# YuQiao0303/PointDreamer

Hardware: AMD Instinct MI355X
Metric: shapes/hour (30k-pt cloud, 8x256^2 views, DDNM) on MI355X (higher is better)
Workload: dtype f16 (f32 accumulate; f32 GroupNorm/softmax statistics, f32 geometry); 1 GPU; configs[2]: synthetic 30k-point sphere shape, 8x256^2 views, texture_gen_method='DDNM_inpaint' (100 DDNM steps, 552.8M-param guided-diffusion UNet, random-init weights), NBF [21], atlas 1024^2, complete_unseen_by='unproject', optimize_from=None, hidden-point removal on (device); 4 independent shapes per step, their views batched through the UNet together; parallelism=shapes-parallel x1, views_per_unet_batch=32

## Files before the change

include/pdhip.h:

```cpp
#ifndef PDHIP_H
#define PDHIP_H
#include <stdint.h>
#include <stddef.h>
#ifdef __cplusplus
extern "C" {
#endif

#define PDHIP_OK 0
#define PDHIP_E_ARG (-1)
#define PDHIP_E_HIP (-2)
#define PDHIP_E_STATE (-3)
#define PDHIP_E_NOMEM (-4)
#define PDHIP_E_UNKNOWN_NAME (-5)

int pdhip_version(void);
int pdhip_lab_build(void);
const char* pdhip_last_error(void);
int pdhip_debug_carve_log(int on);
int pdhip_debug_carve_log_read(uint64_t* triples, int capacity);

int pdhip_project_points(const float* cam_params, int V, const float* vertices, int Vn,
                         const float* points, int N, int rescale, double padding,
                         float* pos , float* vertice_uvs ,
                         float* uv_centers, float* uv_scales,
                         float* point_uvs , float* point_depths ,
                         uint32_t* minmax_ws, void* stream);

int pdhip_raster_mesh(const float* pos , int V, int Vn, const int32_t* faces , int F,
                      int R, uint64_t* zkey_ws, uint8_t* hard_masks, int64_t* face_idxs, float* depths,
                      void* stream);
size_t pdhip_raster_mesh_ws_bytes(int V, int F, int R);
int pdhip_raster_mesh_ws(const float* pos, int V, int Vn, const int32_t* faces, int F, int R, uint64_t* zkey_ws, size_t ws_bytes,
                         uint8_t* hard_masks, int64_t* face_idxs, float* depths, void* stream);
int pdhip_debug_set_raster_path(int path);

int pdhip_raster_barycentrics(const float* pos , int V, int Vn, const int32_t* faces, int R,
                              const int64_t* face_idxs , float* bary , void* stream);
int pdhip_interpolate(const float* attr , int C, const int32_t* tri , const int64_t* face_idxs,
                      const float* bary, long long pixels, float* out , void* stream);

int pdhip_shade_views(const int64_t* face_idxs , const float* bary , int V, int R, const float* attr ,
                      int Na, int C, const int32_t* tri , int F, const float* atlas , int A,
                      const float* face_normals , const float* cam_params ,
                      const float* light_dirs , int L, int double_side, double gamma, float* images ,
                      uint8_t* rgba , void* stream);

int pdhip_shade_views_materials(const int64_t* face_idxs , const float* bary , int V, int R,
                                const float* uvs , int T, const int64_t* face_uvs_idx ,
                                const int32_t* face_material , int F,
                                const uint8_t* texels , int64_t texel_bytes, const int64_t* mat_offset ,
                                const int32_t* mat_wh , const float* mat_kd , int M,
                                const float* face_normals , const float* cam_params ,
                                const float* light_dirs , int L, int double_side, double gamma,
                                float* images , uint8_t* rgba ,
                                int32_t* material_idx , void* stream);

size_t pdhip_image_metrics_workspace_bytes(int N, int H, int W);
int pdhip_image_metrics(const uint8_t* a, const uint8_t* b, int N, int H, int W, int C, int gaussian, uint64_t* sse ,
                        double* ssim , void* ws, void* stream);

size_t pdhip_uv_atlas_ws_bytes(int Vn, int F);
int pdhip_uv_atlas(const float* vertices , int Vn, const int64_t* faces , int F, int resolution, int gutter,
                   float* uvs , int64_t* tex_idx , int32_t* face_chart ,
                   int32_t* counts ,
                   void* ws, void* stream);

size_t pdhip_estimate_normals_ws_bytes(int N, int k, int n_eyes);
int pdhip_estimate_normals(const float* points , int N, int k, int n_eyes, double eye_radius, float* normals ,
                           int32_t* counts , void* ws, void* stream);
size_t pdhip_surface_recon_ws_bytes(int N, int depth);
int pdhip_surface_recon(const float* points , const float* normals , const float* colors , int N, int depth,
                        float* vertices, int vertex_capacity, int64_t* faces, int face_capacity, float* vertex_colors ,
                        int32_t* counts , float* info , void* ws, void* stream);

size_t pdhip_simplify_mesh_workspace_bytes(int Vn, int F);
int pdhip_simplify_mesh(const float* vertices , int Vn, const int64_t* faces , int F, const float* vertex_colors ,
                        int target_faces, float* out_vertices , int64_t* out_faces , float* out_colors ,
                        int32_t* counts , void* ws, void* stream);

size_t pdhip_sample_mesh_workspace_bytes(int F, int N);
int pdhip_sample_mesh(const float* vertices , int Vn, const int64_t* faces , int F, const float* uvs , int T,
                      const int64_t* face_uvs_idx , const int32_t* face_material ,
                      const uint8_t* face_keep , const uint8_t* texels , int64_t texel_bytes,
                      const int64_t* mat_offset , const int32_t* mat_wh , const float* mat_kd , int M,
                      const float* rand , int N, float* coords , float* colors , float* normals ,
                      float* uvs_out , int32_t* face_idx , int32_t* material_idx , void* ws, void* stream);

int pdhip_project_points_shapes(const float* cam_params , int V, int S, const float* vertices , int Vn,
                                const float* points , int N, int rescale, double padding, float* pos ,
                                float* vertice_uvs, float* uv_centers , float* uv_scales , float* point_uvs ,
                                float* point_depths , uint32_t* minmax_ws , void* stream);
int pdhip_raster_mesh_shapes(const float* pos , int V, int S, int Vn, const int32_t* faces , int F, int R,
                             uint64_t* zkey_ws, size_t ws_bytes , uint8_t* hard_masks,
                             int64_t* face_idxs, float* depths, void* stream);
int pdhip_hidden_point_removal_shapes(const float* points , int N, const double* eyes , int V, int S, double radius,
                                      const uint8_t* skip , uint8_t* visibility ,
                                      void* ws , void* stream);
int pdhip_sparse_views_shapes(const int64_t* point_pixels , const float* colors , const uint8_t* validation,
                              const uint8_t* hard_masks, int V, int S, int N, int res, int point_size, int edge_point_size,
                              double mask_ratio_thresh, float* sparse, float* mask0, float* mask2, float* scale_factors ,
                              float* mask_ratios, void* ws , void* stream);
int pdhip_texel_visibility_shapes(const float* cam_params, int V, int S, const float* gb_pos , const uint8_t* mask ,
                                  int A, const float* uv_centers, const float* uv_scales, double padding, const float* mesh_depths ,
                                  int R, float offset, uint8_t* visibility , void* stream);
int pdhip_nbf_shrink_shapes(const uint8_t* mask , const uint8_t* visibility , int V, int S, int A,
                            const int32_t* kernels, int K, uint8_t* out , uint8_t* ws , void* stream);
int pdhip_view_select_blend_shapes(const float* cam_params, int V, int S, const float* gb_pos, const uint8_t* mask, const int64_t* face_id,
                                   int A, const float* f_normals , int F, const float* base_dirs , const float* uv_centers,
                                   const float* uv_scales, double padding, const float* scale_factors, const uint8_t* shrinked ,
                                   int K, const uint8_t* visibility, int complete_unseen_by_projection, const float* inpainted ,
                                   int r, float* atlas , uint8_t* painted , int32_t* view_ids ,
                                   void* stream);

int pdhip_rescale_vertices(float* pos , int V, int Vn, const float* uv_centers, const float* uv_scales,
                           const float* factors , double padding, void* stream);
size_t pdhip_optimize_color_ws_bytes(int V, int res, int A);
int pdhip_optimize_color(float* atlas, int A, const float* uv_map, const int64_t* face_idxs, int V, int res,
                         const float* inpainted , int r, const uint8_t* shrinked, double lr, int iterations,
                         float* final_images, void* ws, void* stream);

int pdhip_resize_mask(const uint8_t* in , int B, int in_h, int in_w,
                      uint8_t* out , int out_h, int out_w, void* stream);

int pdhip_point_visibility(int cam_res, const float* point_uvs , const float* point_depths ,
                           const float* mesh_depths , int V, int N, float offset,
                           uint8_t* visibility , int64_t* point_pixels , void* stream);

size_t pdhip_hpr_ws_bytes(int V, int N);
int pdhip_hidden_point_removal(const float* points , int N, const double* eyes , int V, double radius,
                               const uint8_t* skip, uint8_t* visibility, void* ws, void* stream);
int pdhip_hpr_read_counters(const void* ws, int V, long long* out , void* stream);

int pdhip_point_pixels(const float* point_uvs , int V, int N, int res,
                       int64_t* point_pixels , void* stream);
int pdhip_point_visibility_pixels(int cam_res, const float* point_uvs, const float* point_depths, const float* mesh_depths,
                                  int V, int N, float offset, uint8_t* visibility , int res,
                                  int64_t* point_pixels , void* stream);

size_t pdhip_sparse_views_ws_bytes(int V, int N, int res);
int pdhip_sparse_views(const int64_t* point_pixels , const float* colors ,
                       const uint8_t* validation , const uint8_t* hard_masks ,
                       int V, int N, int res, int point_size, int edge_point_size, double mask_ratio_thresh,
                       float* sparse , float* mask0, float* mask2,
                       float* scale_factors , float* mask_ratios ,
                       void* ws, void* stream);

size_t pdhip_nearest_fill_ws_ints(int B, int H, int W);
int pdhip_nearest_fill(const float* img, float* out, int B, int C, int H, int W,
                       int64_t batch_stride, int64_t chan_stride, int64_t pix_stride,
                       const void* mask, int mask_is_f32, int64_t mask_batch_stride,
                       int32_t* ws, void* stream);

size_t pdhip_linear_fill_ws_bytes(int B, int H, int W);
int pdhip_linear_fill(const float* img, float* out, int B, int C, int H, int W, const void* mask, int mask_is_f32,
                      int64_t mask_batch_stride, void* ws, int32_t* tri, void* stream);
int pdhip_linear_fill_unresolved(const void* ws, int B, int H, int W, int* out, void* stream);
int pdhip_debug_set_linear_local(int on);

int pdhip_debug_set_unproject_generic(int on);

int pdhip_texel_visibility(const float* cam_params, int V, const float* gb_pos ,
                           const uint8_t* mask , int A, const float* uv_centers ,
                           const float* uv_scales , double padding,
                           const float* mesh_depths , int R, float offset,
                           uint8_t* visibility, void* stream);

int pdhip_nbf_shrink(const uint8_t* mask , const uint8_t* visibility , int V, int A,
                     const int32_t* kernels, int K, uint8_t* out, uint8_t* ws, void* stream);
int pdhip_pack_bits(const uint8_t* in , long long n, uint64_t* out , void* stream);
int pdhip_unpack_bits(const uint64_t* in , long long n, uint8_t* out , void* stream);
int pdhip_nbf_triptych(const uint8_t* mask, const uint8_t* visibility, int V, int A, int kernel, uint8_t* out, uint8_t* ws,
                       void* stream);

int pdhip_view_select_blend(const float* cam_params, int V, const float* gb_pos, const uint8_t* mask,
                            const int64_t* face_id , int A, const float* f_normals ,
                            const float* base_dirs , const float* uv_centers, const float* uv_scales,
                            double padding, const float* scale_factors ,
                            const uint8_t* shrinked, int K, const uint8_t* visibility,
                            int complete_unseen_by_projection,
                            const float* inpainted , int r,
                            float* atlas, uint8_t* painted, int32_t* view_ids, void* stream);

int pdhip_compact_texels(const float* gb_pos, const uint8_t* mask, int A, const int32_t* view_ids,
                         float* points, int64_t* coords, int64_t* point_view_ids, int32_t* count_dev,
                         int32_t* ws, void* stream);

typedef struct pdhip_unet pdhip_unet;

int pdhip_unet_create(int image_size, int model_channels, int num_res_blocks, const int* channel_mult, int n_mult,
                      const int* attention_ds, int n_att, int num_head_channels, int out_channels, int max_batch,
                      pdhip_unet** out);
void pdhip_unet_destroy(pdhip_unet* u);
long long pdhip_unet_arena_bytes(const pdhip_unet* u);
int pdhip_unet_route_table(int image_size, int model_channels, int num_res_blocks, const int* channel_mult, int n_mult, const int* attention_ds,
                           int n_att, int num_head_channels, int out_channels, int max_batch, int N, char* buf, int buf_len);
int pdhip_unet_num_tensors(const pdhip_unet* u);
int pdhip_unet_load_tensor(pdhip_unet* u, const char* name, const void* data, int is_f16, const int64_t* shape, int ndim,
                           void* stream);
int pdhip_unet_missing_tensors(const pdhip_unet* u, char* buf, int buf_len);
int pdhip_unet_forward(pdhip_unet* u, const float* x, const float* t, int N, float* out, void* stream);
int pdhip_unet_profile(pdhip_unet* u, int enable);
int pdhip_unet_profile_read(pdhip_unet* u, double* total_ms, double* total_flops, long long* launches);
int pdhip_unet_profile_read_attention(pdhip_unet* u, double* total_ms, double* total_flops, long long* launches);

int pdhip_ddnm_schedule(float* at, float* at_next, int* t, int* t_next, float* coefs);
int pdhip_ddnm_prepare(const float* masked_imgs , const float* masks , float* y, int N, int HW, void* stream);
int pdhip_ddnm_step(float* x, const float* et, int et_channels, const float* y, const float* mask, const float* eps,
                    uint64_t seed, int step, int N, int HW, void* stream);
int pdhip_ddnm_sample(pdhip_unet* u, const float* masked_imgs, const float* masks, int N, const float* x_T,
                      const float* eps_tape, uint64_t seed, int n_steps, float* out, void* stream);
int pdhip_ddnm_sample_keyed(pdhip_unet* u, const float* masked_imgs, const float* masks, int N, const float* x_T,
                            const float* eps_tape, uint64_t seed, uint64_t first_image_key, int n_steps, float* out, void* stream);

int pdhip_debug_set_conv_bk(int bk);
int pdhip_debug_set_conv_tile(int geometry);
int pdhip_debug_set_conv_stages(int stages);
int pdhip_debug_set_conv_splitk(void* ws, long long ws_floats, int splits);
int pdhip_debug_set_conv_halo_strips(int mode);
int pdhip_pack_conv_weight_f16(const float* w_oihw, int Cout, int Cin, int taps, void* w_packed , void* stream);
int pdhip_conv2d_nhwc_f16(const void* x, const void* w_packed , const float* bias, const void* residual,
                          void* y, int N, int H, int W, int Cin, int Cout, int Cout_pad, int taps, const void* zero_page,
                          void* stream);
int pdhip_groupnorm_nhwc_f16(const void* x, const float* gamma, const float* beta, const float* film , int N,
                             int H, int W, int C, int silu, int resample, void* y, float* stats_ws, float* ws,
                             long long ws_floats, void* stream);
int pdhip_gn_silu_conv3x3_nhwc_f16(const void* x, const float* gamma, const float* beta, const float* film ,
                                   long long film_stride, const void* w_packed, const float* bias, const void* residual, void* y,
                                   int N, int H, int W, int Cin, int Cout, int Cout_pad, const void* zero_page, float* ws,
                                   long long ws_floats, void* stream);
int pdhip_debug_conv3x3_apply(const void* x, const float* table , const void* w_packed, const float* bias, const void* residual,
                              void* y, int N, int H, int W, int Cin, int Cout, int Cout_pad, const void* zero_page, void* stream);
int pdhip_debug_set_fold_skip(int on);
int pdhip_debug_set_up_phase(int mode);
int pdhip_pack_conv_up2_phase_f16(const void* w_packed, int Cin, int Cout_pad, void* w_phase, void* stream);
int pdhip_conv3x3_up2_phase_nhwc_f16(const void* x, const void* w_phase, const float* bias, void* y, int N, int H, int W, int Cin, int Cout,
                                     int Cout_pad, const void* zero_page, float* gn_part, void* stream);
int pdhip_conv3x3_up2_halo_nhwc_f16(const void* x, const void* w_packed, const float* bias, void* y, int N, int H, int W, int Cin, int Cout,
                                    int Cout_pad, const void* zero_page, void* stream);
int pdhip_debug_set_fold_resample(int on);
int pdhip_debug_set_fold_finalize(int max_batch);
int pdhip_debug_set_fold_finalize_chunks(int chunks);
int pdhip_debug_set_conv_sk(int mode, int tile, int splits);
int pdhip_debug_set_conv_sk_stages(int stages);
int pdhip_debug_set_conv_sk_kgroups(int kg);
int pdhip_debug_set_attn(int nbuf, int vt_form, int qtiles);
int pdhip_debug_set_conv_sk_order(int order);
int pdhip_gn_silu_skip1x1_nhwc_f16(const void* xa, const void* xb, int Ca, int C, const float* stats, const float* gamma, const float* beta,
                                   const void* w_packed, const float* bias, void* h0, void* sk, int N, int H, int W, void* stream);
int pdhip_debug_set_gn_iters(int iters);
int pdhip_debug_set_gn_skip_variant(int v);
int pdhip_debug_set_fuse_skip(int mode, int min_tiles);
int pdhip_debug_set_fuse_gn(int on);
int pdhip_mark_unpainted_faces(const int64_t* face_id, const uint8_t* painted, int A, int F, uint8_t* flags , void* stream);
int pdhip_vertex_texel_fetch(const float* vert_uvs , int V, const float* atlas , const uint8_t* mask ,
                             int A, int32_t* texel , float* colors , float* count , void* stream);
int pdhip_neighbor_diffuse_round(const int32_t* rowptr , const int32_t* colidx, int V, const int32_t* invalid, int IV,
                                 float* colors, float* count, float* tmp , int* colored, void* stream);
int pdhip_scatter_vertex_colors(const int32_t* texel, const float* colors, int V, float* atlas, uint8_t* mask,
                                int32_t* owner_ws , int A, void* stream);
size_t pdhip_subdivide_with_uv_ws_bytes(int V, int U, int F, int K);
int pdhip_subdivide_with_uv(const float* vertices , int V, const int64_t* faces , int F, const float* uvs , int U,
                            const int64_t* face_uv_idx , const int64_t* face_index , int K,
                            float* out_vertices, int64_t* out_faces, float* out_uvs, int64_t* out_face_uv_idx,
                            int32_t* counts , int32_t* counts_host , void* ws, void* stream);
size_t pdhip_vertex_uv_table_ws_bytes(int V, int F);
int pdhip_vertex_uv_table(int V, const int64_t* faces , const int64_t* face_uv_idx , int F, const float* uvs ,
                          int U, float* vert_uvs , int32_t* counts , void* ws, void* stream);
size_t pdhip_neighbour_csr_ws_bytes(int V, int F);
int pdhip_neighbour_csr(int V, const int64_t* faces , int F, int32_t* rowptr , int32_t* colidx ,
                        int32_t* counts , int32_t* counts_host , void* ws, void* stream);
size_t pdhip_compact_zero_count_ws_bytes(int V);
int pdhip_compact_zero_count(const float* count , int V, int32_t* invalid , int32_t* counts ,
                             int32_t* counts_host , void* ws, void* stream);

long long pdhip_io_ply_count(const char* path);
int pdhip_io_read_ply_xyzrgb(const char* path, float* xyz , uint8_t* rgb , long long n);
int pdhip_io_write_obj_mtl(const char* obj_path, const char* mtl_path, const char* texture_stem, const double* points, long long P,
                           const double* tcoords, long long T, const int64_t* faces, const int64_t* facetex, long long F);
int pdhip_io_write_obj_plain(const char* obj_path, const float* points , long long P, const int64_t* faces , long long F);
int pdhip_io_write_png(const char* path, const uint8_t* hwc, int H, int W, int channels, int zlib_level);
int pdhip_chw_f32_to_hwc_u8(const float* img, int C, int H, int W, uint8_t* out, void* stream);

size_t pdhip_unet_head_ws_floats(int N, int H, int W, int C, int Cout);
int pdhip_unet_head_f32(const void* x, const float* gamma, const float* beta, const float* w_oihw, const float* bias,
                        int N, int H, int W, int C, int Cout, float* y_nchw, float* ws, long long ws_floats, void* stream);
int pdhip_conv_rr_f16(const void* x, const void* x2, int C, int Ca, int gn_mode, const float* gamma, const float* beta, const float* film,
                      long long film_stride, const float* partA, int chunksA, const float* partB, int chunksB, const void* xs, const void* xs2, int Cs,
                      int Cs1, int taps, const void* wf, const float* bias, const void* residual, int res_up, void* y, int N, int H, int W, int Cout,
                      float* ws, long long ws_floats, float* gn_part, int* gn_chunks, void* stream);
long long pdhip_conv_rr_weight_halfs(int Cin, int taps, int Cs, int Cout);
int pdhip_conv_rr_pack_f16(const void* w_packed, int Cin, int taps, int Cs, int Cout, void* wf, void* stream);
int pdhip_gn_octet_partials_f16(const void* x, int N, int HW, int C, int chunks, float* part, void* stream);
int pdhip_gn_apply_parts_f16(const void* x, const void* x2, int Ca, int C, const float* partA, int chunksA, const float* partB, int chunksB, const float* gamma,
                             const float* beta, const float* film, long long film_stride, int N, int H, int W, int silu, void* y, void* stream);
int pdhip_debug_conv_launch_nhwc_f16(const void* x, const void* x2, int Cin1, const void* w_packed, const float* bias, const void* residual, int res_up,
                                     const void* xs, const void* xs2, int Cs1, int Cs, void* y, int N, int H, int W, int Cin, int Cout, int Cout_pad, int taps,
                                     const void* zero_page, float* ws, long long ws_floats, float* gn_part, long long gn_part_floats, int* gn_chunks, int* kernel,
                                     void* stream);
int pdhip_gn_finalize_oct_f32(const float* partA, int Ca, int chunksA, const float* partB, int Cb, int chunksB, int N, int HW, float* stats, void* stream);
int pdhip_conv_ht_f16(const void* x, const void* w_packed, const float* bias, const void* residual, int res_up, void* y, int N, int H, int W, int Cin, int Cout,
                      int Cout_pad, const void* zero_page, float* splitk_ws, long long splitk_ws_floats, float* gn_part, int* gn_chunks, void* stream);
int pdhip_conv_ht_plan(int N, int H, int W, int Cin, int Cout, int Cout_pad, long long splitk_ws_floats, int* routed, int* slabs);
int pdhip_debug_set_conv_ht(int mode, int slabs);
int pdhip_debug_set_rr_gn(int max_width);
int pdhip_debug_set_conv_rr(int mode, int variant, int slabs);
int pdhip_attention_f16(const void* qkv , void* out , int N, int T, int C, int head_dim,
                        void* vt_ws , void* stream);
int pdhip_philox_normal(float* out, long long n, uint64_t seed, uint64_t stream_id, void* stream);
int pdhip_gemv_rows_f32(const float* W, const float* b, const float* x, float* y, int R, int K, int N, int silu_out, void* stream);
int pdhip_timestep_mlp_f32(const float* t, int N, int mc, const float* w0, const float* b0, const float* w2, const float* b2, float* emb_silu,
                           float* tmp, void* stream);
int pdhip_conv_in_f16(const float* x_nchw, const void* Wt, const float* bias, void* Y, int N, int H, int W, int Cout, int Cout_pad, void* im2col_ws,
                      const void* zero_page, void* stream);
int pdhip_gn_apply_f16(const void* x, const void* x2, int Ca, int C, const float* stats, const float* partA, int chunksA, const float* partB, int chunksB,
                       const float* gamma, const float* beta, const float* film, long long film_stride, int N, int H, int W, int silu, int resample, void* y,
                       void* y_raw, void* stream);
int pdhip_gn_table_f32(const float* stats, const float* gamma, const float* beta, const float* film, long long film_stride, int N, int C, float* table, void* stream);
int pdhip_resample2x_nhwc_f16(const void* x, int N, int H, int W, int C, int mode, void* y, void* stream);
int pdhip_concat_channels_f16(const void* a, int Ca, const void* b, int Cb, long long pixels, void* y, void* stream);
int pdhip_bench_copy16(const void* src, void* dst, long long bytes, int blocks, int unroll, void* stream);

size_t pdhip_nearest_points_workspace_bytes(int Q, int M);
int pdhip_nearest_points_stage_chunk(void);
int pdhip_nearest_points(const float* queries, int Q, const float* targets, int M, double* d2, int32_t* idx, int32_t* counts, void* ws, void* stream);
int pdhip_debug_set_nearest_path(int path);
size_t pdhip_cloud_metrics_workspace_bytes(int T);
int pdhip_cloud_metrics(const double* d2, const int32_t* idx, int Q, const float* normals_src, const float* normals_tgt, int M,
                        const double* thresholds, int T, double* sums, int64_t* within, void* ws, void* stream);

size_t pdhip_mesh_contains_workspace_bytes(int Vn, int F, int Q, int resolution);
int pdhip_mesh_contains(const float* vertices, int Vn, const int64_t* faces, int F, const float* points, int Q, int resolution, uint8_t* occ,
                        int32_t* counts, void* ws, void* stream);
int pdhip_debug_set_mesh_contains_slabs(int slabs);
int pdhip_occupancy_iou(const uint8_t* a, const uint8_t* b, int Q, int64_t* out, void* stream);

size_t pdhip_closest_on_mesh_workspace_bytes(int Vn, int F, int Q);
int pdhip_closest_on_mesh(const float* vertices, int Vn, const int64_t* faces, int F, const float* points, int Q, double* d2, int32_t* face,
                          double* closest, int32_t* counts, void* ws, void* stream);
int pdhip_debug_set_closest_on_mesh(int cells_per_axis, int path);

size_t pdhip_fps_workspace_bytes(int N, int M);
int pdhip_fps(const float* points, int N, int M, int start, int32_t* idx, double* min_d2, int32_t* counts, void* ws, void* stream);
int pdhip_debug_set_fps_cells(int cells_per_axis);
size_t pdhip_owner_mean_colors_workspace_bytes(int M);
int pdhip_owner_mean_colors(const int32_t* owner, const float* colors, int N, int M, const float* fallback, float* out, void* ws_or_null, void* stream);

size_t pdhip_knn_points_workspace_bytes(int Q, int M, int k);
int pdhip_knn_max_k(void);
size_t pdhip_knn_lds_bytes(int k);
int pdhip_knn_points(const float* queries, int Q, const float* targets, int M, int k, double* d2, int32_t* idx, int32_t* counts, void* ws, void* stream);
int pdhip_debug_set_knn(int cells_per_axis, int path);
size_t pdhip_sor_filter_workspace_bytes(int N);
int pdhip_sor_filter(const double* knn_d2, int N, int kk, double std_ratio, double* mean_d, double* stats, uint8_t* keep, int32_t* kept_idx,
                     int32_t* counts, void* ws, void* stream);

size_t pdhip_mesh_components_workspace_bytes(int Vn, int F);
int pdhip_mesh_components(const int64_t* faces, int F, const float* vertices_or_null, int Vn, int32_t* vertex_comp, int32_t* face_comp,
                          int32_t* comp_root, int32_t* comp_vertices, int32_t* comp_faces, float* comp_box_or_null, int comp_capacity,
                          int32_t* counts, void* ws, void* stream);
size_t pdhip_compact_mesh_workspace_bytes(int Vn, int F);
int pdhip_compact_mesh(const float* vertices, int Vn, const int64_t* faces, int F, const float* colors_or_null, const uint8_t* face_keep,
                       float* out_vertices, int64_t* out_faces, float* out_colors_or_null, int32_t* vertex_map_or_null, int32_t* counts, void* ws,
                       void* stream);

int pdhip_mesh_boundary_vertices(const int64_t* faces, int F, int Vn, const int32_t* rowptr, const int32_t* colidx, int32_t* pair_faces,
                                 uint8_t* boundary, int32_t* counts, void* stream);
int pdhip_smooth_mesh(const float* vertices, int Vn, const int32_t* rowptr, const int32_t* colidx, const uint8_t* held_or_null, int steps,
                      double lambda, double mu, double* state_a, double* state_b, float* out_vertices, int32_t* counts, void* stream);

#ifdef __cplusplus
}
#endif
#endif
```

pointdreamer_amd/csrc/nn_common.h:

```cpp
#pragma once
#include "common.h"
#include <hip/hip_fp16.h>

namespace pdnn {

typedef _Float16 half_t;
typedef __attribute__((ext_vector_type(8))) _Float16 half8;
typedef __attribute__((ext_vector_type(4))) _Float16 half4;
typedef __attribute__((ext_vector_type(4))) float float4_t;

struct Tuning {
    int force_bk = 0;
    int force_stages = 0;
    int force_wmw = 0;
    int force_splits = 0;
    int halo_strips = 0;
    int sk_mode = 1;
    int sk_tile = 0;
    int sk_splits = 0;
    int sk_stages = 0;
    int sk_kg = 0;
    int sk_order = 0;
    int rr_mode = 1;
    int rr_variant = 0;
    int rr_slabs = 0;
    int ht_mode = 1;
    int ht_slabs = 0;
    int fuse_gn = 0;
    int fold_resample = 1;
    int fold_skip = 1;
    int rr_gn = 0;
    int fold_finalize = 8, fold_finalize_chunks = 16;
    int fuse_skip = 1, fuse_skip_min_tiles = 1;
    int up_phase = 1;
    int attn_nbuf = 0;
    int attn_qtn = 0;
    int attn_vt = 0;
    int gn_iters = 0;
    int gs_variant = 1;
};
Tuning& tuning();

bool conv3x3_halo_eligible(int N, int H, int W, int Cin, int Cout_pad);
int conv3x3_halo_splits(int N, int H, int W, int Cin, int Cout, int Cout_pad, size_t splitk_ws_floats);
int conv3x3_halo_launch_splits(const Tuning& t, int N, int H, int W, int Cin, int Cout, int Cout_pad, size_t halo_ws_floats);
inline bool conv3x3_halo_rows(const Tuning& t, int H, int W) { return W == 256 && (t.halo_strips == 1 || H % 4 != 0); }
int conv3x3_halo(const half_t* X, const half_t* Wt, const float* bias, const half_t* residual, half_t* Y, int N, int H, int W,
                 int Cin, int Cout, int Cout_pad, const half_t* zero_page, hipStream_t s, float* gn_part, int splits, bool full_rows,
                 float* splitk_ws, size_t splitk_ws_floats, const float* apply_table = nullptr, int res_up = 0,
                 int in_up = 0);
int splitk_reduce(const float* partial, int splits, long long M, int Cout, const float* bias, const half_t* residual, half_t* Y,
                  float* gn_part, int hw, hipStream_t s);
int conv_igemm(const Tuning& t, const half_t* X, const half_t* Wt, const float* bias, const half_t* residual, half_t* Y, int N, int H,
               int W, int Cin, int Cout, int Cout_pad, int taps, const half_t* zero_page, hipStream_t s,
               float* splitk_ws = nullptr, size_t splitk_ws_floats = 0, float* gn_part = nullptr,
               const half_t* X2 = nullptr, int Cin1 = 0,
               const float* apply_table = nullptr,
               int res_up = 0,
               int in_up = 0);
bool conv_up2_phase_eligible(int N, int H, int W, int Cin, int Cout, int Cout_pad);
int conv_up2_phase_pack(const half_t* w9, int Cin, int Cout_pad, half_t* dst, hipStream_t s);
int conv_up2_phase(const half_t* X, const half_t* Wph, const float* bias, half_t* Y, int N, int H, int W, int Cin, int Cout, int Cout_pad,
                   const half_t* zero_page, hipStream_t s, float* gn_part, int geo);
struct SkPlan { int bm, bn, splits, tile_id;
                int kg, stages, m_fast; };
SkPlan conv_sk_plan(const Tuning& t, int N, int H, int W, int Cin, int Cout, int Cout_pad, int taps, bool two_source, size_t ws_floats, int k_extra = 0);
int conv_sk_skip(const SkPlan& pl, const half_t* X, const half_t* Wt, const float* bias, half_t* Y, int N, int H, int W, int Cin, int Cout,
                 int Cout_pad, const half_t* XS, const half_t* XS2, int Cs1, int Cs, const half_t* zero_page, hipStream_t s, float* ws,
                 size_t ws_floats, float* gn_part);
int fuse_skip_weights(const half_t* w3, int K9, const half_t* w1, int Cs, int Cout_pad, const float* b3, const float* b1, int Cout, half_t* dst,
                      float* bdst, hipStream_t s);
int conv_sk(const SkPlan& pl, const half_t* X, const half_t* Wt, const float* bias, const half_t* residual, half_t* Y, int N, int H, int W,
            int Cin, int Cout, int Cout_pad, int taps, const half_t* zero_page, hipStream_t s, float* ws, size_t ws_floats, float* gn_part,
            const half_t* X2, int Cin1, int res_up = 0);
#define PD_SK_TICKET_FLOATS 4096
int gn_finalize_oct(const float* partA, int Ca, int chunksA, const float* partB, int Cb, int chunksB, int N, int HW, float eps,
                    float* stats, hipStream_t s);

struct RrIn {
    const half_t* x; const half_t* x2; int C, Ca;
    int gn;
    const float* gamma; const float* beta; const float* film; long long film_stride;
    const float* partA; const float* partB; int chunksA, chunksB; float eps;
};
struct RrPlan { int variant, S0, U0, S1, U1, bands, ntiles; };
RrPlan conv_rr_plan(const Tuning& t, int N, int H, int W, int Cin, int Cout, int taps, int Cs , size_t ws_floats,
                    bool want_gn = false );
size_t conv_rr_weight_halfs(int Cin, int taps, int Cs, int Cout);
int conv_rr_pack(const half_t* w_packed, int Cin, int taps, int Cs, int Cout, half_t* dst, hipStream_t s);
int conv_rr(const RrPlan& pl, const RrIn& in, const RrIn* skip, int taps, const half_t* wf, const float* bias, const half_t* residual, int res_up,
            half_t* Y, int N, int H, int W, int Cout, float* ws, size_t ws_floats, float* gn_part , hipStream_t s);
#define PD_RR_MAX_PART_LOADS 8

bool conv_ht_routes(const Tuning& t, int N, int H, int W, int Cin, int Cout, int Cout_pad, size_t ws_floats);
int conv_ht_slabs(const Tuning& t, int N, int H, int W, int Cin, int Cout_pad, size_t ws_floats);
int conv_ht(const half_t* X, const half_t* Wt, const float* bias, const half_t* residual, half_t* Y, int N, int H, int W, int Cin, int Cout,
            int Cout_pad, const half_t* zero_page, hipStream_t s, float* gn_part , int res_up, int slabs, float* ws, size_t ws_floats);

enum ConvKernel { CONV_HALO, CONV_RR, CONV_HT, CONV_SK, CONV_IGEMM, CONV_UP_PHASE };
const char* conv_kernel_name(ConvKernel k);
struct ConvNeeds {
    bool two_source = false;
    bool in_up = false;
    bool apply = false;
    bool in_gn = false;
    bool want_gn = false;
    int skip_cs = 0;
    bool have_wf = false, have_wf_skip = false;
};
struct ConvPlan {
    int N = 0, H = 0, W = 0, Cin = 0, Cout = 0, Cout_pad = 0, taps = 0;
    ConvKernel kernel = CONV_IGEMM;
    SkPlan sk{0, 0, 0, 0}; RrPlan rr{0, 0, 0, 0, 0, 0, 0};
    int splits = 1;
    bool halo_rows = false;
    int slabs = 1;
    int bk = 0, geo = 0;
    int stages = 0;
    bool want_gn = false;
    int gn_chunks = 0;
    bool takes_res_up = false;
    bool takes_in_up = false, takes_apply = false, takes_in_gn = false, takes_skip = false;
    int skip_cs = 0;
};
ConvPlan conv_plan(const Tuning& t, int N, int H, int W, int Cin, int Cout, int Cout_pad, int taps, const ConvNeeds& needs, size_t ws_floats);
ConvPlan conv_up2_phase_plan(const Tuning& t, int N, int H, int W, int Cin, int Cout, int Cout_pad, bool want_gn);
struct ConvArgs {
    const half_t* X; const half_t* X2; int Cin1;
    const half_t* Wt;
    const float* bias; const half_t* residual; int res_up;
    const float* apply_table;
    const RrIn* rr_in;
    const half_t* XS; const half_t* XS2; int Cs1;
    half_t* Y; const half_t* zero_page; float* ws; size_t ws_floats;
    float* gn_part;
};
int conv_launch(const ConvPlan& p, const ConvArgs& a, hipStream_t s);

__device__ __forceinline__ float silu_f(float x) { return x * __builtin_amdgcn_rcpf(1.0f + __expf(-x)); }

__device__ __forceinline__ float gn_round_f16(float f) { asm("" : "+v"(f)); return (float)(half_t)f; }
template <bool OUT_F32, bool FILM>
__device__ __forceinline__ float gn_elem(float x, float ga, float gb, float t1, float sh, int silu) {
    float f = __builtin_fmaf(x, ga, gb);
    if (!OUT_F32) f = gn_round_f16(f);
    if (FILM) {
        f = gn_round_f16(f * t1);
        f = gn_round_f16(f + sh);
    }
    if (silu) { f = silu_f(f); if (!OUT_F32) f = gn_round_f16(f); }
    return f;
}


int gn_stats(const half_t* X, int N, int HW, int C, float eps, float* stats, float* ws, size_t ws_floats, hipStream_t s);
struct GnPartsArg { const float* partA; int Ca, chunksA; const float* partB; int Cb, chunksB; float eps; };
int gn_apply(const half_t* X, const float* stats, const float* gamma, const float* beta, const float* film,
             long long film_stride, int N, int H, int W, int C, int silu, int resample, void* Y, int out_f32, hipStream_t s,
             const half_t* XB = nullptr, int Ca = 0,
             half_t* Yraw = nullptr,
             const GnPartsArg* parts = nullptr,
             int iters_hook = 0);
int gn_table(const float* stats, const float* gamma, const float* beta, const float* film, long long film_stride, int N, int C,
             float* table, hipStream_t s);
bool gn_skip_eligible(int N, int HW, int Ca, int C, int Cout, int Cout_pad);
int gn_skip(const half_t* XA, const half_t* XB, int Ca, int C, const float* stats, const float* gamma, const float* beta, const half_t* Wt,
            const float* bias, half_t* H0, half_t* SK, int N, int HW, hipStream_t s, int variant );
int resample2x(const half_t* X, int N, int H, int W, int C, int mode, half_t* Y, hipStream_t s);
int concat_channels(const half_t* A, int Ca, const half_t* B, int Cb, long long pixels, half_t* Y, hipStream_t s);

int attention(const half_t* qkv, half_t* out, int N, int T, int C, int D, hipStream_t s, half_t* vt_ws, int nbuf, int qtn, int vt);

int conv_in_3x3(const ConvPlan& p, const float* x_nchw, const half_t* Wt , const float* bias, half_t* Y,
                int N, int H, int W, int Cout, int Cout_pad, half_t* im2col_ws , const half_t* zero_page, hipStream_t s, float* gn_part = nullptr);
int head_pack(const float* w, int NO, int C, half_t* wz, hipStream_t s);
int head_gn_silu_conv3x3(const half_t* X, const float* stats, const float* gamma, const float* beta, const half_t* wz,
                         const float* bias, float* y_nchw, int N, int H, int W, int C, int NO, hipStream_t s);
int timestep_mlp(const float* t, int N, int mc, const float* w0, const float* b0, const float* w2, const float* b2,
                 float* emb_silu , float* tmp, hipStream_t s);
int gemv_rows(const float* Wm , const float* b, const float* x , float* y , int R, int K, int N,
              hipStream_t s);

struct DdnmCoef { float sqrt_1m_at, sqrt_at, sqrt_at_next, sigma_t, c1, c2; };
int ddnm_update(float* x , const float* et , int Cet, const float* y,
                const float* mask , const float* eps , unsigned long long seed,
                unsigned long long step, DdnmCoef co, int N, int HW, hipStream_t s, unsigned long long quad0 = 0);
int ddnm_prepare(const float* masked_img, const float* mask, float* y, int N, int HW, hipStream_t s);
int ddnm_finish(const float* x, float* out, long long n, hipStream_t s);
int copy16(const void* src, void* dst, long long bytes, int blocks, int unroll, hipStream_t s);
int philox_normal(float* out, long long n, unsigned long long seed, unsigned long long stream_id, hipStream_t s,
                  unsigned long long quad0 = 0);

}
```

pointdreamer_amd/csrc/nn_conv_halo.hip:

```cpp
#include <type_traits>
#include "nn_common.h"
using namespace pdhip;
namespace pdnn {
namespace {

typedef __attribute__((address_space(3))) void lds_void_h;
typedef const __attribute__((address_space(1))) void gbl_void_h;
__device__ __forceinline__ void glds16h(const void* gsrc, void* lds_wave_base) {
#ifndef PD_LAB_NODMA
    __builtin_amdgcn_global_load_lds((gbl_void_h*)gsrc, (lds_void_h*)lds_wave_base, 16, 0, 0);
#endif
}
__device__ __forceinline__ int swz_b(int row) { return (0x78 >> (2 * ((row >> 2) & 3))) & 3; }
__device__ __forceinline__ int swz_a(int hp) { return ((hp >> 2) & 1) << 1; }

template <int WLOG, int ILOG, bool APPLY>
__global__ __launch_bounds__(512) void k_conv3x3_halo(const half_t* __restrict__ X, const half_t* __restrict__ Wt,
                                                      const float* __restrict__ bias, const half_t* __restrict__ residual,
                                                      half_t* __restrict__ Y, int N, int H, int Cin, int Cout, int n_tiles,
                                                      int total_tiles, const half_t* __restrict__ zero_page,
                                                      float* __restrict__ gn_part, int splits, float* __restrict__ partial,
                                                      const float* __restrict__ ap_table, int res_up, int in_up) {
    constexpr int W = 1 << WLOG, BMT = 512, BNT = 128, TM = 8, ROWB = 64, NWAVES = 8;
    constexpr int RT = BMT / W, HW2 = W + 2, HP = (RT + 2) * HW2;
    constexpr int NPA = (HP + 15) / 16, PA = (NPA + 7) / 8;
    constexpr int AH_BYTES = NPA * 1024, B_BYTES = BNT * ROWB;
    constexpr int RPW = W >= 128 ? 1 : 128 / W;
    constexpr int FPR = TM / RPW;
    constexpr int CS_LD = BNT + 8;
    static_assert(PA <= 9 && RPW <= 4, "halo schedule: at most one halo piece per wave per tap, W >= 32");
    static_assert(!APPLY || PA <= 7, "APPLY: piece T-1 is finished under step T+1 <= 8");
    constexpr int SCR_OFF = 2 * AH_BYTES + 3 * B_BYTES;
    constexpr int TAB_OFF = SCR_OFF + NWAVES * 1024;
    extern __shared__ __attribute__((aligned(16))) char smem[];
    const int tid = threadIdx.x, lane = tid & 63;
    const int wave = __builtin_amdgcn_readfirstlane(tid >> 6);
    const int wm = wave >> 1, wn = wave & 1;
    int tile;
    {
        const int b = blockIdx.x, q = total_tiles >> 3, r = total_tiles & 7, xcd = b & 7, i = b >> 3;
        tile = (xcd < r ? xcd * (q + 1) : r * (q + 1) + (xcd - r) * q) + i;
    }
    const int pt = tile / n_tiles, n0 = (tile % n_tiles) * BNT;
    const int HWp = H << ILOG;
    const int tpi = HWp / BMT;
    const int img = pt / tpi, tin = pt - img * tpi;
    constexpr int STRIPS = 1 << (ILOG - WLOG);
    const int ty0 = (tin / STRIPS) * RT, x0 = (tin % STRIPS) << WLOG;
    auto pix = [&](int p) -> long long { return (((long long)img * H + ty0 + (p >> WLOG)) << ILOG) + x0 + (p & (W - 1)); };
    const int K = 9 * Cin;
    const int NCT = Cin >> 5;
    const int cb = (int)((long long)NCT * blockIdx.y / splits), NC = (int)((long long)NCT * (blockIdx.y + 1) / splits) - cb;

    constexpr int PA_TAB = PA > 6 ? 6 : PA;
    const int cq = lane & 3;
    auto halo_off = [&](int t) -> uint32_t {
        const int pi = min(t * 8 + wave, NPA - 1);
        int lq = lane >> 2;
        asm volatile("" : "+v"(lq));
        const int hp = pi * 16 + lq;
        const int hy = hp / HW2, hx = hp - hy * HW2;
        const int y = ty0 - 1 + hy, x = x0 + hx - 1;
        const bool ok = (hp < HP) & (y >= 0) & (y < H) & (x >= 0) & (x < (1 << ILOG));
        const int spix = ((img * (H >> in_up) + (y >> in_up)) << (ILOG - in_up)) + (x >> in_up);
        return ok ? (uint32_t)((spix * Cin + ((cq ^ swz_a(hp)) << 3)) * 2) : ~0u;
    };
    uint32_t aoff[PA_TAB];
#pragma unroll
    for (int t = 0; t < PA_TAB; ++t) aoff[t] = halo_off(t);
    const char* const Xb = reinterpret_cast<const char*>(X);
    auto halo_src = [&](int t, int chunk) -> const void* {
        uint32_t off = t < PA_TAB ? aoff[t < PA_TAB ? t : 0] : halo_off(t);
        if constexpr (APPLY) asm volatile("" : "+v"(off));
        return off == ~0u ? (const void*)zero_page : (const void*)(Xb + off + (uint32_t)chunk * 64u);
    };
    const int brow = wave * 16 + (lane >> 2);
    const half_t* bp = Wt + (size_t)(n0 + brow) * K + cb * 32 + (((lane & 3) ^ swz_b(brow)) << 3);
    char* const ah_dst = smem;
    char* const b_dst = smem + 2 * AH_BYTES + wave * 1024;
    auto piece_off = [&](int t, int buf) -> int {
        const int pi = t * 8 + wave;
        if (APPLY) return pi < NPA ? buf * AH_BYTES + pi * 1024 : SCR_OFF + wave * 1024;
        return buf * AH_BYTES + min(pi, NPA - 1) * 1024;
    };

    const int r16 = lane & 15, q4 = lane >> 4;
    const uint32_t lds0 = (uint32_t)(uintptr_t)(__attribute__((address_space(3))) char*)smem;
    const int p0 = wm * 128;
    const int hp0 = ((p0 >> WLOG) + 1) * HW2 + (p0 & (W - 1)) + 1 + r16;
    const uint32_t b_frag = lds0 + 2 * AH_BYTES + (wn * 64 + r16) * ROWB + ((q4 ^ swz_b(r16)) << 4);
    float4_t acc[TM][4];
#pragma unroll
    for (int i = 0; i < TM; ++i)
#pragma unroll
        for (int j = 0; j < 4; ++j) acc[i][j] = (float4_t){0.f, 0.f, 0.f, 0.f};

#define HL_DSR(dst, addr, off) asm volatile("ds_read_b128 %0, %1 offset:%2" : "=v"(dst) : "v"(addr), "n"(off))
#define HL_AADDR(buf, toff, row2)                                                                                    \
    (lds0 + (buf) * AH_BYTES + (uint32_t)((hpv + (toff) + (row2) * HW2) << 6) + (uint32_t)((q4 ^ swz_a(hpv + (toff) + (row2) * HW2)) << 4))
    half8 ar[4], bf[2][4];

    half8 ap_d;
    int ap_k = 0;
    uint32_t ap_lds = 0;
    uint32_t ap_v = 0;
    const int ap_o = wave & 3, ap_h = wave >> 2;
    const uint32_t val_lds = lds0 + (uint32_t)TAB_OFF + (uint32_t)Cin * 8u;
    auto ap_fetch = [&](int t, int buf) {
        int hp = ap_h * 64 + lane;
        asm volatile("" : "+v"(hp));
        hp += t * 128;
        const bool real = hp < NPA * 16;
        ap_lds = real ? lds0 + (uint32_t)(buf * AH_BYTES) + ((uint32_t)hp << 6) + (uint32_t)((ap_o ^ swz_a(hp)) << 4)
                      : lds0 + (uint32_t)SCR_OFF + (uint32_t)(wave * 1024 + lane * 16);
#ifndef PD_LAB_AP_NOFETCH
        HL_DSR(ap_d, ap_lds, 0);
        asm volatile("ds_read_u8 %0, %1" : "=v"(ap_v) : "v"(val_lds + (uint32_t)(real ? hp : 0)));
#endif
    };
    auto ap_consts = [&](int chunk) {
        asm volatile("ds_read_b32 %0, %1" : "=v"(ap_k) : "v"(lds0 + (uint32_t)TAB_OFF + (uint32_t)(((chunk * 4 + ap_o) * 16 + (lane & 15)) << 2)));
    };
    auto ap_pair = [&](int j) {
#ifdef PD_LAB_AP_NOCOMPUTE
        return;
#endif
        int kk = ap_k;
        asm volatile("" : "+v"(kk));
#pragma unroll
        for (int e = 2 * j; e < 2 * j + 2; ++e) {
            const float A = __builtin_bit_cast(float, __builtin_amdgcn_readlane(kk, e));
            const float B = __builtin_bit_cast(float, __builtin_amdgcn_readlane(kk, 8 + e));
            float y = (float)ap_d[e] * A + B;
#ifndef PD_LAB_AP_NOTRANS
            y = y * __builtin_amdgcn_rcpf(1.0f + __expf(-y));
#endif
            ap_d[e] = (half_t)y;
        }
    };
    auto ap_store = [&]() {
        typedef __attribute__((ext_vector_type(4))) uint32_t u32x4;
        u32x4 v = __builtin_bit_cast(u32x4, ap_d);
        const bool ok = ap_v != 0;
        v[0] = ok ? v[0] : 0u; v[1] = ok ? v[1] : 0u; v[2] = ok ? v[2] : 0u; v[3] = ok ? v[3] : 0u;
#ifndef PD_LAB_AP_NOSTORE
        asm volatile("ds_write_b128 %0, %1" :: "v"(ap_lds), "v"(v) : "memory");
#endif
    };

#pragma unroll
    for (int t = 0; t < PA; ++t) glds16h(halo_src(t, cb), ah_dst + piece_off(t, 0));
    glds16h(bp, b_dst);
    bp += Cin;
    glds16h(bp, b_dst + B_BYTES);
    bp += Cin;
    if (PA == 9) {
        glds16h(halo_src(PA - 1, cb), ah_dst + piece_off(PA - 1, 0));
#ifndef PD_LAB_NOPROWAIT
        asm volatile("s_waitcnt vmcnt(2)" ::: "memory");
#endif
    } else {
#ifndef PD_LAB_NOPROWAIT
        asm volatile("s_waitcnt vmcnt(1)" ::: "memory");
#endif
    }
    if constexpr (APPLY) {
        const float4_t* tg = reinterpret_cast<const float4_t*>(ap_table) + (size_t)img * (Cin >> 1);
        float4_t* tl = reinterpret_cast<float4_t*>(smem + TAB_OFF);
        for (int i = tid; i < (Cin >> 1); i += NWAVES * 64) tl[i] = tg[i];
        uint8_t* vl = reinterpret_cast<uint8_t*>(smem + TAB_OFF) + (size_t)Cin * 8;
        for (int hp = tid; hp < NPA * 16; hp += NWAVES * 64) {
            const int hy = hp / HW2, hx = hp - hy * HW2;
            const int y = ty0 - 1 + hy, x = x0 + hx - 1;
            vl[hp] = ((hp < HP) & (y >= 0) & (y < H) & (x >= 0) & (x < (1 << ILOG))) ? 1 : 0;
        }
        asm volatile("s_waitcnt vmcnt(0) lgkmcnt(0)" ::: "memory");
        __builtin_amdgcn_s_barrier();
        asm volatile("" ::: "memory");
        ap_consts(cb);
#pragma unroll
        for (int t = 0; t < PA; ++t) {
            ap_fetch(t, 0);
            asm volatile("s_waitcnt lgkmcnt(0)" : "+v"(ap_d), "+v"(ap_v), "+v"(ap_k));
            ap_pair(0); ap_pair(1); ap_pair(2); ap_pair(3);
            ap_store();
        }
        asm volatile("s_waitcnt lgkmcnt(0)" ::: "memory");
    }
    __builtin_amdgcn_s_barrier();
    asm volatile("" ::: "memory");
    {
        const int hpv = hp0;
        const uint32_t a0 = HL_AADDR(0, -HW2 - 1, 0);
        HL_DSR(bf[0][0], b_frag, 0); HL_DSR(bf[0][1], b_frag, 16 * ROWB); HL_DSR(bf[0][2], b_frag, 32 * ROWB); HL_DSR(bf[0][3], b_frag, 48 * ROWB);
        HL_DSR(ar[0], a0, 0); HL_DSR(ar[1], a0, 1024);
        if constexpr (FPR > 2) { HL_DSR(ar[2], a0, 2048); } else { const uint32_t a1 = HL_AADDR(0, -HW2 - 1, 1); HL_DSR(ar[2], a1, 0); }
    }

    int bs = 0;
    uint32_t a_carry;
    { const int hpv = hp0; a_carry = HL_AADDR(0, -HW2 - 1, 0); }
    const int S = 9 * NC;
    for (int c0 = 0; c0 < NC; c0 += 2) {
#ifdef PD_LAB_AP_LOOSEVM
#define HL_VMN(T) (1 + ((T) < PA ? 1 : 0) + (((((T) + 8) % 9) < PA) ? 1 : 0))
#else
#define HL_VMN(T) (1 + ((T) < PA ? 1 : 0) + ((!APPLY && (((T) + 8) % 9) < PA) ? 1 : 0))
#endif
#define HL_GROUP(P, T, g)                                                                                              \
    {                                                                                                                 \
        if constexpr ((g) + 3 < TM) {                                  \
            if constexpr (RPW > 1 && ((g) == 0 || ((g) + 3) % FPR == 0 || RPW == 2))                                  \
                a_cur = HL_AADDR(ab, (T / 3 - 1) * HW2 + (T % 3 - 1), ((g) + 3) / FPR);                               \
            HL_DSR(ar[((g) + 3) & 3], a_cur, (((g) + 3) % FPR) * 1024);                                               \
        }                                                                                                             \
        if constexpr ((g) == 5) {                                                                                     \
            if (more) {                                                                                               \
                asm volatile("s_waitcnt vmcnt(%3) lgkmcnt(0)" : "+v"(ar[1]), "+v"(ar[2]), "+v"(ar[3]) : "n"(HL_VMN(T)) : "memory"); \
                __builtin_amdgcn_s_barrier();                                                                         \
                asm volatile("" ::: "memory");                                                                        \
                const uint32_t b_nx = b_frag + (bs == 2 ? 0 : bs + 1) * B_BYTES;                                      \
                a_nx0 = HL_AADDR(abn, dyn_ * HW2 + dxn_, 0);                                                          \
                a_carry = a_nx0;                                                                                      \
                HL_DSR(bf[bn][0], b_nx, 0); HL_DSR(bf[bn][1], b_nx, 16 * ROWB);                                       \
                HL_DSR(bf[bn][2], b_nx, 32 * ROWB); HL_DSR(bf[bn][3], b_nx, 48 * ROWB);                               \
                HL_DSR(ar[0], a_nx0, 0);                                                                              \
                if constexpr (APPLY && (T) >= 1 && (T) - 1 < PA) {     \
                    if constexpr ((T) == 1) ap_consts(cb + min(c + 1, NC - 1));                                       \
                    ap_fetch((T) - 1, ab ^ 1);                                                                        \
                }                                                                                                     \
            } else {                                                                                                  \
                asm volatile("s_waitcnt lgkmcnt(0)" : "+v"(ar[1]), "+v"(ar[2]), "+v"(ar[3]));                         \
            }                                                                                                         \
        } else if constexpr ((g) == 6) {                                                                              \
            if (more) HL_DSR(ar[1], a_nx0, 1024);                                                                     \
        } else if constexpr ((g) == 7) {                                                                              \
            if (more) {                                                                                               \
                if constexpr (FPR == 2) a_nx0 = HL_AADDR(abn, dyn_ * HW2 + dxn_, 1);                                  \
                HL_DSR(ar[2], a_nx0, (2 % FPR) * 1024);                                                               \
            }                                                                                                         \
        } else {                                                                                                      \
            asm volatile("s_waitcnt lgkmcnt(3)" : "+v"(ar[(g) & 3]));                                                 \
            if constexpr ((g) == 0) asm volatile("" : "+v"(bf[bc][0]), "+v"(bf[bc][1]), "+v"(bf[bc][2]), "+v"(bf[bc][3])); \
            if constexpr (APPLY && (g) == 0 && (T) >= 2 && (T) - 2 < PA)    \
                asm volatile("" : "+v"(ap_d), "+v"(ap_v), "+v"(ap_k));                                                \
        }                                                                                                             \
        if constexpr (APPLY && (T) >= 2 && (T) - 2 < PA) {              \
            if constexpr ((g) <= 3) ap_pair(g);                                                                       \
            else if constexpr ((g) == 4) ap_store();                                                                  \
        }                                                                                                             \
        _Pragma("unroll") for (int j = 0; j < 4; ++j)                                                                 \
            acc[g][j] = __builtin_amdgcn_mfma_f32_16x16x32_f16(bf[bc][j], ar[(g) & 3], acc[g][j], 0, 0, 0);           \
        if constexpr ((g) == 0) {                                          \
            const int st2 = bs == 0 ? 2 : bs - 1;                                                                     \
            if (s + 2 < S) {                                                                                          \
                glds16h(bp, b_dst + st2 * B_BYTES);                                                                   \
                if constexpr (((T) + 2) % 9 < 8) bp += Cin; else bp += 32 - 8 * Cin;                                  \
            } else glds16h(zero_page, b_dst + st2 * B_BYTES);            \
        }                                                                                                             \
        if constexpr ((g) == 1 && (T) < PA) {                                          \
            glds16h(halo_src(T, cb + min(c + 1, NC - 1)), ah_dst + piece_off(T, ab ^ 1));                            \
        }                                                                                                             \
        __builtin_amdgcn_sched_barrier(0);                                                                            \
    }
#define HL_STEP(P, T)                                                                                                 \
    {                                                                                                                 \
        constexpr int tn_ = ((T) + 1) % 9;                                                                            \
        constexpr int dyn_ = tn_ / 3 - 1, dxn_ = tn_ % 3 - 1;                                                         \
        constexpr int ab = (P), bc = ((P) + (T)) & 1, bn = bc ^ 1;     \
        const int s = c * 9 + (T);                                                                                    \
        const bool more = s + 1 < S;                                                                                  \
        int hpv = hp0;                                                                                                \
        asm volatile("" : "+v"(hpv));                                  \
        uint32_t a_cur = a_carry;                                      \
        const int abn = (T) == 8 ? (ab ^ 1) : ab;                                                                     \
        uint32_t a_nx0 = 0;                                            \
        HL_GROUP(P, T, 0) HL_GROUP(P, T, 1) HL_GROUP(P, T, 2) HL_GROUP(P, T, 3)                                        \
        HL_GROUP(P, T, 4) HL_GROUP(P, T, 5) HL_GROUP(P, T, 6) HL_GROUP(P, T, 7)                                        \
        bs = bs == 2 ? 0 : bs + 1;                                                                                    \
    }
#define HL_CHUNK(P) HL_STEP(P, 0) HL_STEP(P, 1) HL_STEP(P, 2) HL_STEP(P, 3) HL_STEP(P, 4) HL_STEP(P, 5) HL_STEP(P, 6) HL_STEP(P, 7) HL_STEP(P, 8)
        { const int c = c0; HL_CHUNK(0) }
        if (c0 + 1 < NC) { const int c = c0 + 1; HL_CHUNK(1) }
#undef HL_CHUNK
#undef HL_STEP
#undef HL_GROUP
#undef HL_VMN
    }
#undef HL_AADDR
#undef HL_DSR
    asm volatile("s_waitcnt vmcnt(0)" ::: "memory");
    __syncthreads();

    if (partial != nullptr) {
        const long long M = (long long)N * HWp;
        float* P = partial + (size_t)blockIdx.y * (size_t)M * Cout;
#pragma unroll
        for (int j = 0; j < 4; ++j) {
            const int n = n0 + wn * 64 + j * 16 + (lane >> 4) * 4;
#pragma unroll
            for (int i = 0; i < TM; ++i) {
                const long long m = pix(wm * TM * 16 + i * 16 + (lane & 15));
                if (n < Cout) *reinterpret_cast<float4_t*>(P + (size_t)m * Cout + n) = acc[i][j];
            }
        }
        return;
    }
#ifdef PD_LAB_NOEPI
    if (pt != -12345) { if (acc[0][0][0] == 123.456f) Y[0] = (half_t)1.f; return; }
#endif
    half_t* Cs = reinterpret_cast<half_t*>(smem);
    constexpr int CT = BNT / 8;
    constexpr int RPP = NWAVES * 64 / CT;
    const int col8 = (tid % CT) * 8;
    float gs = 0.f, gq = 0.f;
    auto epilogue = [&](auto has_res) {
        constexpr bool RES = decltype(has_res)::value;
        float4_t bvs[4];
#pragma unroll
        for (int j = 0; j < 4; ++j) {
            const int nl = wn * 64 + j * 16 + (lane >> 4) * 4;
            bvs[j] = (float4_t){0.f, 0.f, 0.f, 0.f};
            if (bias != nullptr && n0 + nl < Cout) bvs[j] = *reinterpret_cast<const float4_t*>(bias + n0 + nl);
        }
        const bool col_ok = n0 + col8 < Cout;
        const int ccol = col_ok ? n0 + col8 : 0;
        constexpr int NRES = BMT / RPP, NR1 = NRES / 2;
        half8 rres[RES ? NRES : 1];
        auto res_load = [&](int p) {
            const int rp = p * RPP + tid / CT;
            const int ry = ty0 + (rp >> WLOG), rx = x0 + (rp & (W - 1));
            const long long rm = res_up ? ((long long)img * (H >> 1) + (ry >> 1)) * ((1 << ILOG) >> 1) + (rx >> 1) : pix(rp);
            rres[p] = *reinterpret_cast<const half8*>(residual + (size_t)rm * Cout + ccol);
        };
        if (RES) {
#pragma unroll
            for (int p = 0; p < NR1; ++p) res_load(p);
        }
#pragma unroll
        for (int j = 0; j < 4; ++j) {
            const int nl = wn * 64 + j * 16 + (lane >> 4) * 4;
            const float4_t bv = bvs[j];
#pragma unroll
            for (int i = 0; i < TM; ++i) {
                const int ml = wm * TM * 16 + i * 16 + (lane & 15);
                half4 h;
#pragma unroll
                for (int r = 0; r < 4; ++r) h[r] = (half_t)(acc[i][j][r] + bv[r]);
                *reinterpret_cast<half4*>(&Cs[ml * CS_LD + nl]) = h;
            }
        }
        if (RES) {
            asm volatile("" ::: "memory");
#pragma unroll
            for (int p = NR1; p < NRES; ++p) res_load(p);
        }
        __syncthreads();
#pragma unroll
        for (int p = 0; p < BMT / RPP; ++p) {
            const int row = p * RPP + tid / CT;
            const long long m = pix(row);
            half8 v = *reinterpret_cast<const half8*>(&Cs[row * CS_LD + col8]);
            const size_t o = (size_t)m * Cout + n0 + col8;
            if (RES) {
                const half8 rv = rres[p];
#pragma unroll
                for (int e = 0; e < 8; ++e) v[e] = (half_t)((float)v[e] + (float)rv[e]);
            }
            if (col_ok) {
#ifndef PD_LAB_HALO_NOSTORE
                *reinterpret_cast<half8*>(Y + o) = v;
#endif
#pragma unroll
                for (int e = 0; e < 8; ++e) { const float f = (float)v[e]; gs += f; gq += f * f; }
            }
        }
    };
    if (residual != nullptr) epilogue(std::true_type{}); else epilogue(std::false_type{});
#ifdef PD_LAB_HALO_NOSTORE
    if (gs == 123.456f && gq == 7.f) Y[0] = (half_t)1.f;
#endif
    if (gn_part != nullptr) {
        __syncthreads();
        float* red = reinterpret_cast<float*>(smem);
        red[tid * 2] = gs; red[tid * 2 + 1] = gq;
        __syncthreads();
        constexpr int SUB = 8;
        static_assert(RPP % SUB == 0, "GroupNorm partial reduce");
        float* red2 = red + NWAVES * 64 * 2;
        if (tid < CT * SUB) {
            const int j = tid % SUB, c = tid / SUB;
            float s1 = 0.f, q1 = 0.f;
#pragma unroll
            for (int r = 0; r < RPP / SUB; ++r) { s1 += red[((r * SUB + j) * CT + c) * 2]; q1 += red[((r * SUB + j) * CT + c) * 2 + 1]; }
            red2[tid * 2] = s1; red2[tid * 2 + 1] = q1;
        }
        __syncthreads();
        if (tid < CT && n0 + tid * 8 < Cout) {
            float s1 = 0.f, q1 = 0.f;
#pragma unroll
            for (int j = 0; j < SUB; ++j) { s1 += red2[(tid * SUB + j) * 2]; q1 += red2[(tid * SUB + j) * 2 + 1]; }
            const int chunks = tpi;
            const int chunk = tin;
            float* dst = gn_part + (((size_t)img * chunks + chunk) * (Cout >> 3) + (n0 >> 3) + tid) * 2;
            dst[0] = s1; dst[1] = q1;
        }
    }
}

template <int WLOG, int ILOG, bool APPLY>
int launch_halo_v(const half_t* X, const half_t* Wt, const float* bias, const half_t* residual, half_t* Y, int N, int H, int Cin,
                  int Cout, int Cout_pad, const half_t* zero_page, hipStream_t s, float* gn_part, int splits, float* partial,
                  const float* ap_table, int res_up, int in_up) {
    constexpr int W = 1 << WLOG, RT = 512 / W, HP = (RT + 2) * (W + 2), NPA = (HP + 15) / 16;
    const size_t loop_bytes = (size_t)2 * NPA * 1024 + 3 * 8192 + (APPLY ? (size_t)8 * 1024 + (size_t)Cin * 8 + (size_t)NPA * 16 + 16 : 0);
    const size_t smem = std::max<size_t>(loop_bytes, (size_t)512 * (128 + 8) * 2);
    PD_REQUIRE(smem <= 160 * 1024, "conv3x3_halo: %zu bytes of LDS (Cin = %d)", smem, Cin);
    auto kern = k_conv3x3_halo<WLOG, ILOG, APPLY>;
    PD_HIP(hipFuncSetAttribute((const void*)kern, hipFuncAttributeMaxDynamicSharedMemorySize, (int)smem));
    const int n_tiles = Cout_pad / 128;
    const int total = (int)(((long long)N * H * (1 << ILOG)) / 512) * n_tiles;
    kern<<<dim3(total, splits), 512, smem, s>>>(X, Wt, bias, residual, Y, N, H, Cin, Cout, n_tiles, total, zero_page, gn_part, splits,
                                                partial, ap_table, res_up, in_up);
    return PDHIP_OK;
}
template <int WLOG, int ILOG = WLOG>
int launch_halo(const half_t* X, const half_t* Wt, const float* bias, const half_t* residual, half_t* Y, int N, int H, int Cin,
                int Cout, int Cout_pad, const half_t* zero_page, hipStream_t s, float* gn_part, int splits, float* partial,
                const float* ap_table, int res_up, int in_up) {
    constexpr int W = 1 << WLOG, RT = 512 / W, HP = (RT + 2) * (W + 2), NPA = (HP + 15) / 16, PA = (NPA + 7) / 8;
    if constexpr (PA <= 7) {
        if (ap_table != nullptr)
            return launch_halo_v<WLOG, ILOG, true>(X, Wt, bias, residual, Y, N, H, Cin, Cout, Cout_pad, zero_page, s, gn_part, splits, partial, ap_table, res_up, in_up);
    } else {
        PD_REQUIRE(ap_table == nullptr, "conv3x3_halo: the full-row 256-wide tile has no APPLY variant");
    }
    return launch_halo_v<WLOG, ILOG, false>(X, Wt, bias, residual, Y, N, H, Cin, Cout, Cout_pad, zero_page, s, gn_part, splits, partial, nullptr, res_up, in_up);
}

}

bool conv3x3_halo_eligible(int N, int H, int W, int Cin, int Cout_pad) {
    return (W == 32 || W == 64 || W == 128 || W == 256) && ((long long)H * W) % 512 == 0 && Cin % 32 == 0 && Cout_pad % 128 == 0 &&
           (long long)N * H * W * Cin * 2 <= 0xfffffff0LL;
}

int conv3x3_halo_splits(int N, int H, int W, int Cin, int Cout, int Cout_pad, size_t splitk_ws_floats) {
    const long long M = (long long)N * H * W;
    const long long tiles = (M / 512) * (Cout_pad / 128);
    if (tiles >= 256) return 1;
    const int nct = Cin / 32;
    int splits = (int)std::min<long long>(std::min<long long>(256 / tiles, nct / 2), 8);
    while (splits > 1 && (size_t)splits * (size_t)M * Cout > splitk_ws_floats) --splits;
    if (splits < 2 || tiles * splits < 128) return 0;
    return splits;
}

int conv3x3_halo_launch_splits(const Tuning& t, int N, int H, int W, int Cin, int Cout, int Cout_pad, size_t ws_floats) {
    int splits = conv3x3_halo_splits(N, H, W, Cin, Cout, Cout_pad, ws_floats);
    if (splits < 1) splits = 1;
    if (t.force_splits >= 1 && ws_floats > 0)
        splits = (int)std::min<size_t>(std::min(t.force_splits, Cin / 32), ws_floats / ((size_t)N * H * W * Cout));
    return splits < 1 ? 1 : splits;
}

int conv3x3_halo(const half_t* X, const half_t* Wt, const float* bias, const half_t* residual, half_t* Y, int N, int H, int W,
                 int Cin, int Cout, int Cout_pad, const half_t* zero_page, hipStream_t s, float* gn_part, int splits, bool full_rows,
                 float* splitk_ws, size_t splitk_ws_floats, const float* apply_table, int res_up, int in_up) {
    PD_REQUIRE(in_up == 0 || (apply_table == nullptr && H % 2 == 0), "conv3x3_halo: an up-sampled input excludes the in-conv GroupNorm");
    PD_REQUIRE(conv3x3_halo_eligible(N, H, W, Cin, Cout_pad), "conv3x3_halo: unsupported geometry (N=%d H=%d W=%d Cin=%d)", N, H, W, Cin);
    PD_REQUIRE(splits >= 1 && splits <= Cin / 32 && (splits == 1 || (splitk_ws != nullptr && (size_t)splits * N * H * W * Cout <= splitk_ws_floats)),
               "conv3x3_halo: %d splits do not fit the layer / the split-K workspace", splits);
    PD_REQUIRE(W != 256 || full_rows || H % 4 == 0, "conv3x3_halo: column strips need H %% 4 == 0 at W = 256");
    PD_REQUIRE(!res_up || (splits == 1 && residual != nullptr && H % 2 == 0), "conv3x3_halo: an up-sampled residual needs the direct (unsplit) epilogue");
    float* partial = splits > 1 ? splitk_ws : nullptr;
    float* gnp = splits > 1 ? nullptr : gn_part;
#define HL_LAUNCH(WL) launch_halo<WL>(X, Wt, bias, residual, Y, N, H, Cin, Cout, Cout_pad, zero_page, s, gnp, splits, partial, apply_table, res_up, in_up)
    int rc;
#define HL_LAUNCH2(WL, IL) launch_halo<WL, IL>(X, Wt, bias, residual, Y, N, H, Cin, Cout, Cout_pad, zero_page, s, gnp, splits, partial, apply_table, res_up, in_up)
    if (W == 256 && !full_rows) rc = HL_LAUNCH2(7, 8);
    else if (W == 256 && apply_table != nullptr) { set_error("conv3x3_halo: APPLY needs H %% 4 == 0 at W = 256"); return PDHIP_E_ARG; }
    else if (W == 256) rc = HL_LAUNCH(8);
    else if (W == 128) rc = HL_LAUNCH(7);
    else if (W == 64) rc = HL_LAUNCH(6);
    else rc = HL_LAUNCH(5);
#undef HL_LAUNCH
#undef HL_LAUNCH2
    if (rc) return rc;
    PD_LAUNCH_CHECK();
    if (splits > 1) return splitk_reduce(partial, splits, (long long)N * H * W, Cout, bias, residual, Y, gn_part, H * W, s);
    return PDHIP_OK;
}

}
```

pointdreamer_amd/csrc/nn_gemm.hip:

```cpp
#include "nn_common.h"
using namespace pdhip;
namespace pdnn {


#ifdef PD_LAB_STAMP
__device__ unsigned long long g_lab_stamps[8 * 4096];
#define PD_STAMP(k) do { if (threadIdx.x == 0 && blockIdx.x < 4096 && blockIdx.y == 0) g_lab_stamps[blockIdx.x * 8 + (k)] = __builtin_readcyclecounter(); } while (0)
#else
#define PD_STAMP(k) do {} while (0)
#endif
typedef __attribute__((address_space(3))) void lds_void;
typedef const __attribute__((address_space(1))) void gbl_void;

__device__ __forceinline__ void glds16(const void* gsrc, void* lds_wave_base) {
#ifndef PD_LAB_NODMA
    __builtin_amdgcn_global_load_lds((gbl_void*)gsrc, (lds_void*)lds_wave_base, 16, 0, 0);
#endif
}

template <int BKT>
__device__ __forceinline__ int swz(int row) {
    if (BKT == 32) return (0x78 >> (2 * ((row >> 2) & 3))) & 3;
    return (row >> 1) & 7;
}
// ... 272 lines not shown
            else asm volatile("s_waitcnt vmcnt(12)" ::: "memory");
        } else asm volatile("s_waitcnt vmcnt(0)" ::: "memory");
#endif
#ifndef PD_LAB_NOBARRIER
        __builtin_amdgcn_s_barrier();
#endif
        asm volatile("" ::: "memory");
        if (it + D < it1) issue(nxt);
        const char* As = smem + cur * STAGE_BYTES + (wm * TM * 16) * ROWB;
        const char* Bs = smem + cur * STAGE_BYTES + TILE_BYTES + (wn * 64) * ROWB;
#pragma unroll
        for (int kk = 0; kk < KSTEPS; ++kk) {
            half8 a[TM], b[4];
#ifdef PD_LAB_NOLDS
#pragma unroll
            for (int j = 0; j < 4; ++j) { b[j] = (half8){(half_t)j, 1, 2, 3, 4, 5, 6, (half_t)lane}; asm volatile("" : "+v"(b[j])); }
#pragma unroll
            for (int i = 0; i < TM; ++i) { a[i] = (half8){(half_t)i, 1, 2, 3, 4, 5, 6, (half_t)kk}; asm volatile("" : "+v"(a[i])); }
#else
#pragma unroll
            for (int j = 0; j < 4; ++j) b[j] = *reinterpret_cast<const half8*>(Bs + j * 16 * ROWB + frag_off[kk]);
#pragma unroll
            for (int i = 0; i < TM; ++i) a[i] = *reinterpret_cast<const half8*>(As + i * 16 * ROWB + frag_off[kk]);
#endif
#pragma unroll
            for (int i = 0; i < TM; ++i)
#pragma unroll
                for (int j = 0; j < 4; ++j) acc[i][j] = __builtin_amdgcn_mfma_f32_16x16x32_f16(b[j], a[i], acc[i][j], 0, 0, 0);
        }
        cur = (cur + 1 == NST) ? 0 : cur + 1;
        nxt = (nxt + 1 == NST) ? 0 : nxt + 1;
    }
    }
    PD_STAMP(2);
    __syncthreads();
#ifdef PD_LAB_NOEPI
    {
        float t = 0.f;
#pragma unroll
        for (int i = 0; i < TM; ++i)
#pragma unroll
            for (int j = 0; j < 4; ++j) t += acc[i][j][0] + acc[i][j][1] + acc[i][j][2] + acc[i][j][3];
        if (t == 123456.789f) Y[0] = (half_t)t;
        return;
    }
#endif

    if (partial != nullptr) {
        float* P = partial + (size_t)blockIdx.y * (size_t)M * Cout;
#pragma unroll
        for (int j = 0; j < 4; ++j) {
            const int n = n0 + wn * 64 + j * 16 + (lane >> 4) * 4;
#pragma unroll
            for (int i = 0; i < TM; ++i) {
                const long long m = (long long)m0 + wm * TM * 16 + i * 16 + (lane & 15);
                if (m < M && n < Cout) *reinterpret_cast<float4_t*>(P + (size_t)m * Cout + n) = acc[i][j];
            }
        }
        return;
    }
    half_t* Cs = reinterpret_cast<half_t*>(smem);
#pragma unroll
    for (int j = 0; j < 4; ++j) {
        const int nl = wn * 64 + j * 16 + (lane >> 4) * 4;
        float4_t bv = (float4_t){0.f, 0.f, 0.f, 0.f};
        if (bias != nullptr && n0 + nl < Cout) bv = *reinterpret_cast<const float4_t*>(bias + n0 + nl);
#pragma unroll
        for (int i = 0; i < TM; ++i) {
            const int ml = wm * TM * 16 + i * 16 + (lane & 15);
            half4 h;
#pragma unroll
            for (int r = 0; r < 4; ++r) h[r] = (half_t)(acc[i][j][r] + bv[r]);
            *reinterpret_cast<half4*>(&Cs[ml * CS_LD + nl]) = h;
        }
    }
    PD_STAMP(3);
    __syncthreads();
    PD_STAMP(4);
    constexpr int CT = BNT / 8;
    constexpr int RPP = NWAVES * 64 / CT;
    const int col8 = (tid % CT) * 8;
    float gs = 0.f, gq = 0.f;
#pragma unroll
    for (int p = 0; p < BMT / RPP; ++p) {
        const int row = p * RPP + tid / CT;
        const long long m = (long long)m0 + row;
        if (m < M && n0 + col8 < Cout) {
            half8 v = *reinterpret_cast<const half8*>(&Cs[row * CS_LD + col8]);
            size_t o = (size_t)m * Cout + n0 + col8;
            if (TAPS == 4) {
                const int hw = H * W, img = (int)(m / hw), rem = (int)(m - (long long)img * hw), y = rem / W, x = rem - y * W;
                o = ((((size_t)img * 2 * H + 2 * y + (phase >> 1)) * 2 * W) + 2 * x + (phase & 1)) * Cout + n0 + col8;
            }
            if (residual != nullptr) {
                const half8 rv = *reinterpret_cast<const half8*>(residual + o);
#pragma unroll
                for (int e = 0; e < 8; ++e) v[e] = (half_t)((float)v[e] + (float)rv[e]);
            }
#ifdef PD_LAB_NOSTORE
            if (v[0] == (half_t)12345.f) *reinterpret_cast<half8*>(Y + o) = v;
#else
            *reinterpret_cast<half8*>(Y + o) = v;
#endif
#pragma unroll
            for (int e = 0; e < 8; ++e) { const float f = (float)v[e]; gs += f; gq += f * f; }
        }
    }
    PD_STAMP(5);
    if (gn_part != nullptr) {
        __syncthreads();
        float* red = reinterpret_cast<float*>(smem);
        red[tid * 2] = gs; red[tid * 2 + 1] = gq;
        __syncthreads();
        if (tid < CT && n0 + tid * 8 < Cout) {
            float s1 = 0.f, q1 = 0.f;
            for (int r = 0; r < RPP; ++r) { s1 += red[(r * CT + tid) * 2]; q1 += red[(r * CT + tid) * 2 + 1]; }
            const int hw = H * W, chunks = (TAPS == 4 ? 4 : 1) * (hw / BMT);
            const int img = m0 / hw, chunk = (TAPS == 4) ? ((m0 - img * hw) / BMT) * 4 + phase : (m0 - img * hw) / BMT;
            float* dst = gn_part + (((size_t)img * chunks + chunk) * (Cout >> 3) + (n0 >> 3) + tid) * 2;
            dst[0] = s1; dst[1] = q1;
        }
    }
}

#define SK_ROWS 16
__global__ __launch_bounds__(256) void k_splitk_reduce(const float* __restrict__ partial, int splits, long long M, int Cout,
                                                       const float* __restrict__ bias, const half_t* __restrict__ residual,
                                                       half_t* __restrict__ Y, float* __restrict__ gn_part, int hw) {
    __shared__ float s_st[4][64][2];
    const int ol = threadIdx.x & 63, q = threadIdx.x >> 6;
    const int oct = blockIdx.y * 64 + ol;
    const bool live = oct < (Cout >> 3);
    const long long m0 = (long long)blockIdx.x * SK_ROWS;
    const size_t MC = (size_t)M * Cout;
    float gs = 0.f, gq = 0.f;
    if (live) {
        float bv[8];
#pragma unroll
        for (int e = 0; e < 8; ++e) bv[e] = bias ? bias[oct * 8 + e] : 0.f;
        float a[SK_ROWS / 4][8];
#pragma unroll
        for (int j = 0; j < SK_ROWS / 4; ++j)
#pragma unroll
            for (int e = 0; e < 8; ++e) a[j][e] = 0.f;
        for (int sp0 = 0; sp0 < splits; sp0 += 4) {
#pragma unroll
            for (int j = 0; j < SK_ROWS / 4; ++j) {
                const long long m = m0 + q + 4 * j;
                if (m < M) {
                    float4 v0[4], v1[4];
#pragma unroll
                    for (int u = 0; u < 4; ++u) {
                        const int sp = min(sp0 + u, splits - 1);
                        const float* src = partial + (size_t)sp * MC + (size_t)m * Cout + (size_t)oct * 8;
                        v0[u] = *reinterpret_cast<const float4*>(src);
                        v1[u] = *reinterpret_cast<const float4*>(src + 4);
                    }
#pragma unroll
                    for (int u = 0; u < 4; ++u) {
                        if (sp0 + u < splits) {
                            a[j][0] += v0[u].x; a[j][1] += v0[u].y; a[j][2] += v0[u].z; a[j][3] += v0[u].w;
                            a[j][4] += v1[u].x; a[j][5] += v1[u].y; a[j][6] += v1[u].z; a[j][7] += v1[u].w;
                        }
                    }
                }
            }
        }
#pragma unroll
        for (int j = 0; j < SK_ROWS / 4; ++j) {
            const long long m = m0 + q + 4 * j;
            if (m >= M) continue;
            const size_t o = (size_t)m * Cout + (size_t)oct * 8;
            half8 v;
#pragma unroll
            for (int e = 0; e < 8; ++e) v[e] = (half_t)(a[j][e] + bv[e]);
            if (residual != nullptr) {
                const half8 rv = *reinterpret_cast<const half8*>(residual + o);
#pragma unroll
                for (int e = 0; e < 8; ++e) v[e] = (half_t)((float)v[e] + (float)rv[e]);
            }
            *reinterpret_cast<half8*>(Y + o) = v;
#pragma unroll
            for (int e = 0; e < 8; ++e) { const float f = (float)v[e]; gs += f; gq += f * f; }
        }
    }
    if (gn_part == nullptr) return;
    s_st[q][ol][0] = gs; s_st[q][ol][1] = gq;
    __syncthreads();
    if (q == 0 && live) {
        gs = (s_st[0][ol][0] + s_st[1][ol][0]) + (s_st[2][ol][0] + s_st[3][ol][0]);
        gq = (s_st[0][ol][1] + s_st[1][ol][1]) + (s_st[2][ol][1] + s_st[3][ol][1]);
        const int chunks = hw / SK_ROWS;
        const long long img = m0 / hw;
        const int chunk = (int)((m0 - img * hw) / SK_ROWS);
        float* dst = gn_part + (((size_t)img * chunks + chunk) * (Cout >> 3) + oct) * 2;
        dst[0] = gs; dst[1] = gq;
    }
}

template <int TAPS, int BKT, int NSTAGE, int WM, int WN, int TM>
static int launch_conv(dim3 grid, size_t smem, hipStream_t s, const half_t* X, const half_t* Wt, const float* bias,
                       const half_t* residual, half_t* Y, int N, int H, int W, int Cin, int Cout, int n_tiles, int total,
                       const half_t* zero_page, int splits, float* partial, float* gnp, const half_t* X2, int Cin1) {
    auto kern = k_conv_igemm<TAPS, BKT, NSTAGE, WM, WN, TM>;
    if (smem > 65536) PD_HIP(hipFuncSetAttribute((const void*)kern, hipFuncAttributeMaxDynamicSharedMemorySize, (int)smem));
    kern<<<grid, WM * WN * 64, smem, s>>>(X, Wt, bias, residual, Y, N, H, W, Cin, Cout, n_tiles, total, zero_page, splits, partial, gnp, X2, Cin1);
    return PDHIP_OK;
}

const char* conv_kernel_name(ConvKernel k) {
    static const char* const names[] = {"halo", "rr", "ht", "sk", "igemm", "phase"};
    return names[k];
}

ConvPlan conv_plan(const Tuning& t, int N, int H, int W, int Cin, int Cout, int Cout_pad, int taps, const ConvNeeds& nd, size_t ws_floats) {
    ConvPlan p;
    p.N = N; p.H = H; p.W = W; p.Cin = Cin; p.Cout = Cout; p.Cout_pad = Cout_pad; p.taps = taps;
    const long long hw = (long long)H * W, M = (long long)N * hw;
    const bool forced = t.force_wmw != 0 || t.force_bk != 0 || t.force_stages != 0 || t.force_splits != 0;
    const bool halo = !nd.two_source && taps == 9 && conv3x3_halo_eligible(N, H, W, Cin, Cout_pad) &&
                      (t.force_wmw == 32 || (!forced && conv3x3_halo_splits(N, H, W, Cin, Cout, Cout_pad, 0) == 1));
    const bool unsplit = halo && conv3x3_halo_splits(N, H, W, Cin, Cout, Cout_pad, ws_floats) == 1;
    const bool strips = W != 256 || H % 4 == 0;
    const bool single3 = taps == 9 && !nd.two_source;
    const size_t part_floats = ws_floats > PD_SK_TICKET_FLOATS ? ws_floats - PD_SK_TICKET_FLOATS : 0;
    auto done = [&](ConvKernel k) {
        p.kernel = k;
        int chunks = 0;
        switch (k) {
        case CONV_HALO:
            p.splits = conv3x3_halo_launch_splits(t, N, H, W, Cin, Cout, Cout_pad, part_floats);
            p.halo_rows = conv3x3_halo_rows(t, H, W);
            chunks = p.splits > 1 ? (hw % 16 == 0 ? (int)(hw / 16) : 0) : (int)(hw / 512);
            p.takes_res_up = unsplit && p.splits == 1 && strips;
            break;
        case CONV_RR: chunks = p.rr.bands; p.takes_res_up = true; break;
        case CONV_HT: p.slabs = conv_ht_slabs(t, N, H, W, Cin, Cout_pad, ws_floats); chunks = (int)(hw / 256); p.takes_res_up = true; break;
        case CONV_SK: chunks = (hw % p.sk.bm == 0 || p.sk.bm == 2 * hw) ? std::max((int)(hw / p.sk.bm), 1) : 0; p.takes_res_up = true; break;
        default: {
            p.bk = (t.force_bk == 32 || Cin % 64 != 0) ? 32 : 64;
            int geo = t.force_wmw;
            if (geo != 2 && geo != 4 && geo != 8 && geo != 16)
                geo = (Cout_pad % 256 == 0 && ((M + 255) / 256) * (Cout_pad / 256) >= 256) ? 8 : 2;
            if (geo == 8 && Cout_pad % 256 != 0) geo = 2;
            p.geo = geo;
            const int bmt = geo == 2 ? 128 : 256, bnt = geo == 8 ? 256 : 128;
            const int total = (int)((M + bmt - 1) / bmt) * (Cout_pad / bnt);
            const int KI = taps * (Cin / p.bk);
            int splits = 1;
            if (part_floats > 0 && taps == 9 && total <= 256) {
                int cap = 8;
                while (cap < 32 && total * cap < 256 && (size_t)(2 * cap) * M * Cout * sizeof(float) <= (size_t)8 << 20) cap *= 2;
                splits = std::min(std::min((512 + total / 2) / total, KI / 2), cap);
                while (splits > 1 && (size_t)splits * M * Cout > part_floats) --splits;
            }
            if (t.force_splits >= 1 && part_floats > 0)
                splits = (int)std::min<size_t>(std::min(t.force_splits, std::max(KI / 2, 1)), part_floats / ((size_t)M * Cout));
            if (splits < 1 || nd.two_source) splits = 1;
            p.splits = splits;
            int stages = t.force_stages ? t.force_stages : (p.bk == 64 ? (geo == 8 ? 12 : 2) : 3);
            const bool pipe = stages == 12 && p.bk == 64 && (geo == 8 || geo == 16);
            if (stages == 12) stages = 2;
            stages = std::min(std::max(stages, 2), 4);
            while (stages > 2 && (size_t)stages * (bmt + bnt) * p.bk * 2 > 160 * 1024) --stages;
            p.stages = pipe ? 12 : stages;
            chunks = splits == 1 ? (hw % bmt == 0 ? (int)(hw / bmt) : 0) : (hw % SK_ROWS == 0 ? (int)(hw / SK_ROWS) : 0);
        }
        }
        p.gn_chunks = nd.want_gn ? chunks : 0;
        return p;
    };
    p.want_gn = nd.want_gn;
    p.takes_apply = nd.apply && halo && strips;
    if (p.takes_apply) return done(CONV_HALO);
    if (nd.skip_cs > 0 && !halo && taps == 9) {
        p.skip_cs = nd.skip_cs;
        if (nd.have_wf_skip) {
            p.rr = conv_rr_plan(t, N, H, W, Cin, Cout, 9, nd.skip_cs, ws_floats);
            if (p.rr.variant != 0) { p.takes_skip = true; return done(CONV_RR); }
        }
        p.sk = conv_sk_plan(t, N, H, W, Cin, Cout, Cout_pad, 9, false, ws_floats, nd.skip_cs);
        if (p.sk.bm > 0) { p.takes_skip = true; return done(CONV_SK); }
        p.skip_cs = 0;
    }
    if (nd.in_gn && nd.have_wf && single3) {
        p.rr = conv_rr_plan(t, N, H, W, Cin, Cout, 9, 0, ws_floats, true);
        if (p.rr.variant != 0) { p.takes_in_gn = true; return done(CONV_RR); }
    }
    p.takes_in_up = nd.in_up && halo && strips;
    if (unsplit) return done(CONV_HALO);
    if (nd.have_wf && single3 && !p.takes_in_up && !unsplit) {
        p.rr = conv_rr_plan(t, N, H, W, Cin, Cout, 9, 0, ws_floats);
        if (p.rr.variant != 0) return done(CONV_RR);
    }
    if (halo) return done(CONV_HALO);
    if (single3 && !forced && conv_ht_routes(t, N, H, W, Cin, Cout, Cout_pad, ws_floats)) return done(CONV_HT);
    if (!forced) {
        p.sk = conv_sk_plan(t, N, H, W, Cin, Cout, Cout_pad, taps, nd.two_source, ws_floats);
        if (p.sk.bm > 0) return done(CONV_SK);
    }
    return done(CONV_IGEMM);
}

ConvPlan conv_up2_phase_plan(const Tuning& t, int N, int H, int W, int Cin, int Cout, int Cout_pad, bool want_gn) {
    ConvPlan p;
    p.N = N; p.H = H; p.W = W; p.Cin = Cin; p.Cout = Cout; p.Cout_pad = Cout_pad; p.taps = 9;
    p.kernel = CONV_UP_PHASE; p.want_gn = want_gn;
    p.geo = Cout_pad % 256 != 0 || t.force_wmw == 16 ? 16 : 8;
    p.gn_chunks = want_gn && ((long long)H * W / 4) % 256 == 0 ? (int)((long long)H * W / 256) : 0;
    return p;
}

int splitk_reduce(const float* partial, int splits, long long M, int Cout, const float* bias, const half_t* residual, half_t* Y,
                  float* gn_part, int hw, hipStream_t s) {
    dim3 gr((unsigned)((M + SK_ROWS - 1) / SK_ROWS), (unsigned)(((Cout >> 3) + 63) / 64));
    k_splitk_reduce<<<gr, 256, 0, s>>>(partial, splits, M, Cout, bias, residual, Y, gn_part, hw);
    PD_LAUNCH_CHECK();
    return PDHIP_OK;
}

int conv_launch(const ConvPlan& p, const ConvArgs& a, hipStream_t s) {
    const int N = p.N, H = p.H, W = p.W, Cin = p.Cin, Cout = p.Cout, Cout_pad = p.Cout_pad, taps = p.taps;
    const long long hw = (long long)H * W, M = (long long)N * hw;
    float* part_ws = a.ws != nullptr && a.ws_floats > PD_SK_TICKET_FLOATS ? a.ws + PD_SK_TICKET_FLOATS : nullptr;
    const size_t part_floats = part_ws != nullptr ? a.ws_floats - PD_SK_TICKET_FLOATS : 0;
    float* gn_part = p.gn_chunks > 0 ? a.gn_part : nullptr;
    switch (p.kernel) {
    case CONV_HALO:
        return conv3x3_halo(a.X, a.Wt, a.bias, a.residual, a.Y, N, H, W, Cin, Cout, Cout_pad, a.zero_page, s, gn_part, p.splits, p.halo_rows, part_ws, part_floats,
                            a.apply_table, a.res_up, p.takes_in_up ? 1 : 0);
    case CONV_RR: {
        const RrIn plain{a.X, nullptr, Cin, Cin, 0, nullptr, nullptr, nullptr, 0, nullptr, nullptr, 0, 0, 1e-5f};
        const RrIn skip{a.XS, a.XS2, p.skip_cs, a.XS2 ? a.Cs1 : p.skip_cs, 0, nullptr, nullptr, nullptr, 0, nullptr, nullptr, 0, 0, 1e-5f};
        return conv_rr(p.rr, p.takes_in_gn ? *a.rr_in : plain, p.takes_skip ? &skip : nullptr, 9, a.Wt, a.bias, a.residual, a.res_up, a.Y, N, H, W, Cout,
                       a.ws, a.ws_floats, gn_part, s);
    }
    case CONV_HT:
        return conv_ht(a.X, a.Wt, a.bias, a.residual, a.Y, N, H, W, Cin, Cout, Cout_pad, a.zero_page, s, gn_part, a.res_up, p.slabs, a.ws, a.ws_floats);
    case CONV_SK:
        return p.takes_skip ? conv_sk_skip(p.sk, a.X, a.Wt, a.bias, a.Y, N, H, W, Cin, Cout, Cout_pad, a.XS, a.XS2, a.XS2 ? a.Cs1 : p.skip_cs, p.skip_cs,
                                           a.zero_page, s, a.ws, a.ws_floats, gn_part)
                            : conv_sk(p.sk, a.X, a.Wt, a.bias, a.residual, a.Y, N, H, W, Cin, Cout, Cout_pad, taps, a.zero_page, s, a.ws, a.ws_floats, gn_part,
                                      a.X2, a.X2 ? a.Cin1 : Cin, a.res_up);
    case CONV_UP_PHASE:
        return conv_up2_phase(a.X, a.Wt, a.bias, a.Y, N, H / 2, W / 2, Cin, Cout, Cout_pad, a.zero_page, s, gn_part, p.geo);
    case CONV_IGEMM: break;
    }
    const half_t *X = a.X, *Wt = a.Wt, *residual = a.residual, *zero_page = a.zero_page, *X2 = a.X2;
    const float* bias = a.bias;
    half_t* Y = a.Y;
    const int Cin1 = X2 ? a.Cin1 : Cin, bk = p.bk, geo = p.geo, splits = p.splits, stages = p.stages;
    PD_REQUIRE(a.res_up == 0, "conv_igemm: an up-sampled residual needs a layer the halo-resident kernel (unsplit), k_conv_rr, k_conv_ht or k_conv_sk takes");
    PD_REQUIRE((bk == 32 || bk == 64) && (stages == 12 || (stages >= 2 && stages <= 4)) && splits >= 1, "conv_igemm: no plan (bk=%d stages=%d splits=%d)", bk, stages, splits);
    PD_REQUIRE(splits == 1 || (part_ws != nullptr && (size_t)splits * M * Cout <= part_floats), "conv_igemm: split-K workspace too small");
    const int bmt = geo == 2 ? 128 : 256, bnt = geo == 8 ? 256 : 128;
    const int m_tiles = (int)((M + bmt - 1) / bmt), n_tiles = Cout_pad / bnt;
    const int total = m_tiles * n_tiles;
    float* partial = splits > 1 ? part_ws : nullptr;
    dim3 grid(total, splits);
    float* gnp = splits == 1 ? gn_part : nullptr;
    const size_t smem = std::max<size_t>((size_t)(stages == 12 ? 2 : stages) * (bmt + bnt) * bk * 2, (size_t)bmt * (bnt + 8) * 2);
    int rc;
#define ARGS grid, smem, s, X, Wt, bias, residual, Y, N, H, W, Cin, Cout, n_tiles, total, zero_page, splits, partial, gnp, X2, Cin1
#define BY_STAGE(T, B, WM_, WN_, TM_)                                                   \
    (stages == 2 ? launch_conv<T, B, 2, WM_, WN_, TM_>(ARGS) : stages == 3 ? launch_conv<T, B, 3, WM_, WN_, TM_>(ARGS) \
                                                              : launch_conv<T, B, 4, WM_, WN_, TM_>(ARGS))
#define BY_STAGE64(T, WM_, WN_, TM_) (stages == 12 ? launch_conv<T, 64, 12, WM_, WN_, TM_>(ARGS) : BY_STAGE(T, 64, WM_, WN_, TM_))
#define BY_GEO(T, B) (geo == 2 ? BY_STAGE(T, B, 2, 2, 4) : geo == 4 ? BY_STAGE(T, B, 4, 2, 4) : geo == 8 ? BY_STAGE(T, B, 2, 4, 8) : BY_STAGE(T, B, 2, 2, 8))
#define BY_GEO64(T) (geo == 2 ? BY_STAGE(T, 64, 2, 2, 4) : geo == 4 ? BY_STAGE(T, 64, 4, 2, 4) : geo == 8 ? BY_STAGE64(T, 2, 4, 8) : BY_STAGE64(T, 2, 2, 8))
    if (taps == 9) rc = (bk == 64) ? BY_GEO64(9) : BY_GEO(9, 32);
    else rc = (bk == 64) ? BY_GEO64(1) : BY_GEO(1, 32);
#undef BY_GEO64
#undef BY_GEO
#undef BY_STAGE64
#undef BY_STAGE
#undef ARGS
    if (rc) return rc;
    if (splits > 1) return splitk_reduce(partial, splits, M, Cout, bias, residual, Y, gn_part, H * W, s);
    PD_LAUNCH_CHECK();
    return PDHIP_OK;
}

int conv_igemm(const Tuning& t, const half_t* X, const half_t* Wt, const float* bias, const half_t* residual, half_t* Y, int N, int H,
               int W, int Cin, int Cout, int Cout_pad, int taps, const half_t* zero_page, hipStream_t s, float* splitk_ws,
               size_t splitk_ws_floats, float* gn_part, const half_t* X2, int Cin1, const float* apply_table, int res_up, int in_up) {
    PD_REQUIRE(taps == 1 || taps == 9, "conv_igemm: taps must be 1 or 9");
    if (X2 == nullptr) Cin1 = Cin;
    PD_REQUIRE(X2 == nullptr || (taps == 1 && Cin1 > 0 && Cin1 < Cin && Cin1 % 64 == 0 && (Cin - Cin1) % 64 == 0),
               "conv_igemm: a two-source input needs a 1x1 conv and channel counts that are multiples of 64");
    PD_REQUIRE(Cin % 32 == 0 && Cout % 8 == 0 && Cout_pad % 128 == 0 && Cout_pad >= Cout,
               "conv_igemm: need Cin %% 32 == 0, Cout %% 8 == 0, padded Cout %% 128 == 0 (Cin=%d Cout=%d pad=%d)", Cin, Cout, Cout_pad);
    if (splitk_ws == nullptr) splitk_ws_floats = 0;
    ConvNeeds nd;
    nd.two_source = X2 != nullptr; nd.in_up = in_up != 0; nd.apply = apply_table != nullptr; nd.want_gn = gn_part != nullptr;
    const ConvPlan p = conv_plan(t, N, H, W, Cin, Cout, Cout_pad, taps, nd, splitk_ws_floats);
    PD_REQUIRE(!nd.in_up || p.takes_in_up, "conv_igemm: an up-sampled input needs a layer the halo-resident kernel takes");
    PD_REQUIRE(res_up == 0 || p.takes_res_up, "conv_igemm: an up-sampled residual needs a layer the halo-resident kernel (unsplit), k_conv_ht or k_conv_sk takes");
    PD_REQUIRE(!nd.apply || p.takes_apply, "conv_igemm: an input transform needs a layer the halo-resident kernel takes");
    const ConvArgs a{X, X2, Cin1, Wt, bias, residual, res_up, apply_table, nullptr, nullptr, nullptr, 0, Y, zero_page, splitk_ws, splitk_ws_floats, gn_part};
    return conv_launch(p, a, s);
}

__global__ void k_pack_up2_phase(const half_t* __restrict__ w9, int Cout_pad, int Cin, half_t* __restrict__ dst) {
    const long long total = 16LL * Cout_pad * Cin;
    for (long long i = blockIdx.x * (long long)blockDim.x + threadIdx.x; i < total; i += (long long)gridDim.x * blockDim.x) {
        const int c = (int)(i % Cin), tap = (int)((i / Cin) & 3);
        const int o = (int)((i / (4LL * Cin)) % Cout_pad), ph = (int)(i / (4LL * Cin * Cout_pad));
        const int py = ph >> 1, px = ph & 1, ty = tap >> 1, tx = tap & 1;
        const int ky0 = py == 0 ? ty : 2 * ty, ky1 = py == 0 ? 2 * ty : ty + 1;
        const int kx0 = px == 0 ? tx : 2 * tx, kx1 = px == 0 ? 2 * tx : tx + 1;
        float sum = 0.f;
        for (int ky = ky0; ky <= ky1; ++ky)
            for (int kx = kx0; kx <= kx1; ++kx) sum += (float)w9[(size_t)o * 9 * Cin + (size_t)(ky * 3 + kx) * Cin + c];
        dst[i] = (half_t)sum;
    }
}
int conv_up2_phase_pack(const half_t* w9, int Cin, int Cout_pad, half_t* dst, hipStream_t s) {
    const long long total = 16LL * Cout_pad * Cin;
    k_pack_up2_phase<<<(int)std::min<long long>((total + 255) / 256, 4096), 256, 0, s>>>(w9, Cout_pad, Cin, dst);
    PD_LAUNCH_CHECK();
    return PDHIP_OK;
}
bool conv_up2_phase_eligible(int N, int H, int W, int Cin, int Cout, int Cout_pad) {
    return N >= 1 && H >= 1 && W >= 1 && Cin % 64 == 0 && Cout % 8 == 0 && Cout_pad % 128 == 0 && Cout_pad >= Cout &&
           ((long long)N * H * W + 255) / 256 * 4 * (Cout_pad / 128) < (1LL << 30);
}
int conv_up2_phase(const half_t* X, const half_t* Wph, const float* bias, half_t* Y, int N, int H, int W, int Cin, int Cout, int Cout_pad,
                   const half_t* zero_page, hipStream_t s, float* gn_part, int geo) {
    PD_REQUIRE(conv_up2_phase_eligible(N, H, W, Cin, Cout, Cout_pad),
               "conv_up2_phase: need Cin %% 64 == 0, Cout %% 8 == 0, padded Cout %% 128 == 0 (Cin=%d Cout=%d pad=%d)", Cin, Cout, Cout_pad);
    PD_REQUIRE(geo == 16 || (geo == 8 && Cout_pad % 256 == 0), "conv_up2_phase: no plan (geo=%d)", geo);
    PD_REQUIRE(gn_part == nullptr || ((long long)H * W) % 256 == 0, "conv_up2_phase: a pixel tile would straddle two images: no fused statistics");
    const int bnt = geo == 8 ? 256 : 128;
    const long long M = (long long)N * H * W;
    const int m_tiles = (int)((M + 255) / 256), n_tiles = Cout_pad / bnt, total = m_tiles * 4 * n_tiles;
    const size_t smem = std::max<size_t>((size_t)2 * (256 + bnt) * 64 * 2, (size_t)256 * (bnt + 8) * 2);
    dim3 grid(total, 1);
    int rc;
    if (geo == 8) rc = launch_conv<4, 64, 12, 2, 4, 8>(grid, smem, s, X, Wph, bias, nullptr, Y, N, H, W, Cin, Cout, n_tiles, total, zero_page, 1, nullptr, gn_part, nullptr, Cin);
    else rc = launch_conv<4, 64, 12, 2, 2, 8>(grid, smem, s, X, Wph, bias, nullptr, Y, N, H, W, Cin, Cout, n_tiles, total, zero_page, 1, nullptr, gn_part, nullptr, Cin);
    if (rc) return rc;
    PD_LAUNCH_CHECK();
    return PDHIP_OK;
}

#ifdef PD_LAB_STAMP
extern "C" int pdhip_lab_read_stamps(unsigned long long* host, int n) {
    return (int)hipMemcpyFromSymbol(host, HIP_SYMBOL(g_lab_stamps), sizeof(unsigned long long) * n);
}
#endif
}
```

pointdreamer_amd/csrc/nn_unet.hip:

```cpp
#include "nn_common.h"
#include <map>
#include <string>
#include <vector>
#include <cmath>
#include <cstring>
using namespace pdhip;
using namespace pdnn;

namespace {

struct ConvW { half_t* w = nullptr; float* b = nullptr; int cin = 0, cout = 0, cout_pad = 0, taps = 0; bool have_w = false, have_b = false;
               half_t* wf = nullptr; half_t* wph = nullptr; bool has_wf = false, has_wph = false; };
struct NormW { float* g = nullptr; float* b = nullptr; int c = 0; bool have_g = false, have_b = false; };
struct ResB { std::string name; int cin, cout, mode; NormW n1, n2; ConvW c1, c2, skip; long long emb_off; bool has_skip; bool have_ew = false, have_eb = false;
              half_t* c2s_w = nullptr; float* c2s_b = nullptr; bool c2s_ready = false; half_t* c2s_wf = nullptr; int hw = 0; bool has_c2s = false, has_c2s_wf = false; };
struct AttB { std::string name; int c; NormW n; ConvW qkv, proj; };
struct Block { int kind; int idx; };

struct Act { half_t* p; int C, H, W; const float* gn_part = nullptr; int gn_chunks = 0; const float* gn_partB = nullptr; int Ca = 0; int gn_chunksB = 0;
             half_t* p2 = nullptr;
             int row = -1, rowB = -1; };

}
namespace pdnn {
// ... 606 lines not shown
extern "C" int pdhip_unet_route_table(int image_size, int model_channels, int num_res_blocks, const int* channel_mult, int n_mult,
                                      const int* attention_ds, int n_att, int num_head_channels, int out_channels, int max_batch, int N,
                                      char* buf, int buf_len) {
    pdhip_unet u;
    int rc = build_graph(&u, image_size, model_channels, num_res_blocks, channel_mult, n_mult, attention_ds, n_att, num_head_channels, out_channels, max_batch);
    if (rc == PDHIP_OK && (N < 1 || N > max_batch)) { set_error("pdhip_unet_route_table: batch %d outside [1, %d]", N, max_batch); rc = PDHIP_E_ARG; }
    if (rc != PDHIP_OK) return rc;
    u.arena = reinterpret_cast<char*>((size_t)1 << 20);
    u.arena_bytes = ~(size_t)0 >> 1;
    Table table;
    rc = forward_impl(tuning(), &u, nullptr, nullptr, N, nullptr, nullptr, false, nullptr, 0, &table);
    if (rc != PDHIP_OK) return rc;
    std::string all;
    for (const std::string& l : table.line) { all += l; all += '\n'; }
    if (buf && buf_len > 0) { strncpy(buf, all.c_str(), buf_len - 1); buf[buf_len - 1] = 0; }
    return (int)all.size();
}

extern "C" int pdhip_unet_missing_tensors(const pdhip_unet* u, char* buf, int buf_len) {
    if (!u) return -1;
    std::vector<std::string> miss;
    auto conv = [&](const std::string& n, const ConvW& c) { if (!c.have_w) miss.push_back(n + ".weight"); if (!c.have_b) miss.push_back(n + ".bias"); };
    auto norm = [&](const std::string& n, const NormW& c) { if (!c.have_g) miss.push_back(n + ".weight"); if (!c.have_b) miss.push_back(n + ".bias"); };
    if (!u->have_win) miss.push_back("input_blocks.0.0.weight");
    if (!u->have_bin) miss.push_back("input_blocks.0.0.bias");
    const char* te[4] = {"time_embed.0.weight", "time_embed.0.bias", "time_embed.2.weight", "time_embed.2.bias"};
    for (int i = 0; i < 4; ++i) if (!u->have_te[i]) miss.push_back(te[i]);
    for (const ResB& rb : u->res) {
        norm(rb.name + ".in_layers.0", rb.n1); conv(rb.name + ".in_layers.2", rb.c1);
        if (!rb.have_ew) miss.push_back(rb.name + ".emb_layers.1.weight");
        if (!rb.have_eb) miss.push_back(rb.name + ".emb_layers.1.bias");
        norm(rb.name + ".out_layers.0", rb.n2); conv(rb.name + ".out_layers.3", rb.c2);
        if (rb.has_skip) conv(rb.name + ".skip_connection", rb.skip);
    }
    for (const AttB& ab : u->att) { norm(ab.name + ".norm", ab.n); conv(ab.name + ".qkv", ab.qkv); conv(ab.name + ".proj_out", ab.proj); }
    norm("out.0", u->out_norm);
    if (!u->have_ow) miss.push_back("out.2.weight");
    if (!u->have_ob) miss.push_back("out.2.bias");
    if (buf && buf_len > 0) {
        std::string s;
        for (const std::string& m : miss) { if ((int)(s.size() + m.size() + 2) >= buf_len) break; s += m; s += '\n'; }
        strncpy(buf, s.c_str(), buf_len - 1); buf[buf_len - 1] = 0;
    }
    return (int)miss.size();
}

extern "C" int pdhip_unet_num_tensors(const pdhip_unet* u) {
    if (!u) return -1;
    int n = 2 + 4 + 4;
    for (const ResB& rb : u->res) n += 10 + (rb.has_skip ? 2 : 0);
    n += 6 * (int)u->att.size();
    return n;
}

extern "C" int pdhip_unet_load_tensor(pdhip_unet* u, const char* name_c, const void* data, int is_f16, const int64_t* shape,
                                      int ndim, void* stream) {
    PD_REQUIRE(u && name_c && data && shape && ndim >= 1 && ndim <= 4, "pdhip_unet_load_tensor: bad arguments");
    u->steps_cached = 0;
    hipStream_t s = as_stream(stream);
    const std::string name(name_c);
    long long numel = 1;
    for (int i = 0; i < ndim; ++i) numel *= shape[i];
    auto want = [&](long long n, const char* what) -> int {
        PD_REQUIRE(numel == n, "pdhip_unet_load_tensor: %s: %s expects %lld elements, got %lld", name_c, what, n, numel);
        return PDHIP_OK;
    };
    auto load_vec = [&](float* dst, long long n, bool* flag, int round16) -> int {
        PD_TRY(want(n, "vector"));
        k_copy_f32<<<grid_for(n), 256, 0, s>>>(data, is_f16, n, dst, round16);
        PD_LAUNCH_CHECK();
        *flag = true;
        return PDHIP_OK;
    };
    auto load_conv_w = [&](ConvW& c) -> int {
        PD_TRY(want((long long)c.cout * c.cin * c.taps, "conv weight"));
        PD_REQUIRE(shape[0] == c.cout && shape[1] == c.cin, "pdhip_unet_load_tensor: %s: shape mismatch", name_c);
        k_pack_conv<<<grid_for(numel), 256, 0, s>>>(data, is_f16, c.cout, c.cin, c.taps, c.w);
        PD_LAUNCH_CHECK();
        if (c.has_wf) PD_TRY(conv_rr_pack(c.w, c.cin, c.taps, 0, c.cout, c.wf, s));
        if (c.has_wph) PD_TRY(conv_up2_phase_pack(c.w, c.cin, c.cout_pad, c.wph, s));
        c.have_w = true;
        return PDHIP_OK;
    };
    auto ends = [&](const std::string& suf) { return name.size() >= suf.size() && name.compare(name.size() - suf.size(), suf.size(), suf) == 0; };
    auto starts = [&](const std::string& pre) { return name.compare(0, pre.size(), pre) == 0; };
    if (name == "input_blocks.0.0.weight") {
        const int c0 = u->mult[0] * u->mc;
        PD_TRY(want((long long)c0 * 27, "input conv weight"));
        k_pack_conv_in<<<grid_for(numel), 256, 0, s>>>(data, is_f16, c0, u->w_in);
        PD_LAUNCH_CHECK();
        u->have_win = true;
        return PDHIP_OK;
    }
    if (name == "input_blocks.0.0.bias") return load_vec(u->b_in, u->mult[0] * u->mc, &u->have_bin, 1);
    if (name == "time_embed.0.weight") return load_vec(u->te_w0, (long long)u->ted * u->mc, &u->have_te[0], 0);
    if (name == "time_embed.0.bias") return load_vec(u->te_b0, u->ted, &u->have_te[1], 0);
    if (name == "time_embed.2.weight") return load_vec(u->te_w2, (long long)u->ted * u->ted, &u->have_te[2], 0);
    if (name == "time_embed.2.bias") return load_vec(u->te_b2, u->ted, &u->have_te[3], 0);
    if (name == "out.0.weight") return load_vec(u->out_norm.g, u->final_ch, &u->out_norm.have_g, 0);
    if (name == "out.0.bias") return load_vec(u->out_norm.b, u->final_ch, &u->out_norm.have_b, 0);
    if (name == "out.2.bias") return load_vec(u->out_b, u->out_ch, &u->have_ob, 0);
    if (name == "out.2.weight") {
        PD_TRY(want((long long)u->out_ch * u->final_ch * 9, "out conv weight"));
        k_pack_conv_f32<<<grid_for(numel), 256, 0, s>>>(data, is_f16, u->out_ch, u->final_ch, 9, u->out_w);
        PD_LAUNCH_CHECK();
        PD_TRY(head_pack(u->out_w, u->out_ch, u->final_ch, u->head_wz, s));
        PD_TRY(head_pack(u->out_w, 3, u->final_ch, u->head_wz3, s));
        u->have_ow = true;
        return PDHIP_OK;
    }
    for (ResB& rb : u->res) {
        if (!starts(rb.name + ".")) continue;
        const std::string rest = name.substr(rb.name.size() + 1);
        if (rest == "in_layers.0.weight") return load_vec(rb.n1.g, rb.cin, &rb.n1.have_g, 0);
        if (rest == "in_layers.0.bias") return load_vec(rb.n1.b, rb.cin, &rb.n1.have_b, 0);
        if (rest == "in_layers.2.weight") return load_conv_w(rb.c1);
        if (rest == "in_layers.2.bias") return load_vec(rb.c1.b, rb.cout, &rb.c1.have_b, 1);
        if (rest == "emb_layers.1.weight") return load_vec(u->emb_w + rb.emb_off * u->ted, (long long)2 * rb.cout * u->ted, &rb.have_ew, 0);
        if (rest == "emb_layers.1.bias") return load_vec(u->emb_b + rb.emb_off, 2 * rb.cout, &rb.have_eb, 0);
        if (rest == "out_layers.0.weight") return load_vec(rb.n2.g, rb.cout, &rb.n2.have_g, 0);
        if (rest == "out_layers.0.bias") return load_vec(rb.n2.b, rb.cout, &rb.n2.have_b, 0);
        auto refuse = [&](int rc) -> int {
            if (rc != PDHIP_OK || !rb.has_c2s) return rc;
            rb.c2s_ready = false;
            if (rb.c2.have_w && rb.c2.have_b && rb.skip.have_w && rb.skip.have_b && rb.skip.taps == 1) {
                PD_TRY(fuse_skip_weights(rb.c2.w, 9 * rb.c2.cin, rb.skip.w, rb.skip.cin, rb.c2.cout_pad, rb.c2.b, rb.skip.b, rb.cout, rb.c2s_w, rb.c2s_b, s));
                if (rb.has_c2s_wf) PD_TRY(conv_rr_pack(rb.c2s_w, rb.c2.cin, 9, rb.skip.cin, rb.cout, rb.c2s_wf, s));
                rb.c2s_ready = true;
            }
            return PDHIP_OK;
        };
        if (rest == "out_layers.3.weight") return refuse(load_conv_w(rb.c2));
        if (rest == "out_layers.3.bias") return refuse(load_vec(rb.c2.b, rb.cout, &rb.c2.have_b, 1));
        if (rb.has_skip && rest == "skip_connection.weight") return refuse(load_conv_w(rb.skip));
        if (rb.has_skip && rest == "skip_connection.bias") return refuse(load_vec(rb.skip.b, rb.cout, &rb.skip.have_b, 1));
    }
    for (AttB& ab : u->att) {
        if (!starts(ab.name + ".")) continue;
        const std::string rest = name.substr(ab.name.size() + 1);
        if (rest == "norm.weight") return load_vec(ab.n.g, ab.c, &ab.n.have_g, 0);
        if (rest == "norm.bias") return load_vec(ab.n.b, ab.c, &ab.n.have_b, 0);
        if (rest == "qkv.weight") return load_conv_w(ab.qkv);
        if (rest == "qkv.bias") return load_vec(ab.qkv.b, 3 * ab.c, &ab.qkv.have_b, 1);
        if (rest == "proj_out.weight") return load_conv_w(ab.proj);
        if (rest == "proj_out.bias") return load_vec(ab.proj.b, ab.c, &ab.proj.have_b, 1);
    }
    (void)ends;
    set_error("pdhip_unet_load_tensor: unknown tensor name '%s'", name_c);
    return PDHIP_E_UNKNOWN_NAME;
}

extern "C" int pdhip_unet_forward(pdhip_unet* u, const float* x, const float* t, int N, float* out, void* stream) {
    PD_REQUIRE(u && x && t && out, "pdhip_unet_forward: null argument");
    PD_REQUIRE(N >= 1 && N <= u->max_batch, "pdhip_unet_forward: batch %d outside [1, %d]", N, u->max_batch);
    return forward_impl(tuning(), u, x, t, N, out, as_stream(stream), false);
}

extern "C" int pdhip_unet_profile(pdhip_unet* u, int enable) {
    PD_REQUIRE(u, "pdhip_unet_profile: null handle");
    u->prof.on = enable != 0;
    u->prof.period = enable > 1 ? enable : 1;
    u->prof.forwards = 0;
    u->prof.armed = false;
    u->prof.used = 0;
    u->prof.flops[0] = u->prof.flops[1] = 0;
    return PDHIP_OK;
}
static int prof_read(pdhip_unet* u, int cls, double* total_ms, double* total_flops, long long* launches) {
    double ms = 0;
    long long n = 0;
    for (size_t i = 0; i + 1 < u->prof.used; i += 2) {
        if (u->prof.cls[i] != cls) continue;
        PD_HIP(hipEventSynchronize(u->prof.ev[i + 1]));
        float e = 0;
        PD_HIP(hipEventElapsedTime(&e, u->prof.ev[i], u->prof.ev[i + 1]));
        ms += e; ++n;
    }
    *total_ms = ms; *total_flops = u->prof.flops[cls]; *launches = n;
    return PDHIP_OK;
}
extern "C" int pdhip_unet_profile_read(pdhip_unet* u, double* total_ms, double* total_flops, long long* launches) {
    PD_REQUIRE(u && total_ms && total_flops && launches, "pdhip_unet_profile_read: null argument");
    return prof_read(u, 0, total_ms, total_flops, launches);
}
extern "C" int pdhip_unet_profile_read_attention(pdhip_unet* u, double* total_ms, double* total_flops, long long* launches) {
    PD_REQUIRE(u && total_ms && total_flops && launches, "pdhip_unet_profile_read_attention: null argument");
    return prof_read(u, 1, total_ms, total_flops, launches);
}

namespace {
struct Sched { std::vector<int> t; std::vector<DdnmCoef> co; std::vector<float> ab; };
Sched make_schedule() {
    Sched s;
    s.ab.resize(1001);
    double acc = 1.0;
    s.ab[0] = 1.0f;
    const double b0 = 1e-4, b1 = 0.02, step = (b1 - b0) / 999.0;
    for (int i = 0; i < 1000; ++i) {
        const double beta = (i == 999) ? b1 : b0 + (double)i * step;
        acc = acc * (double)(1.0f - (float)beta);
        s.ab[i + 1] = (float)acc;
    }
    const double eta = 0.85;
    for (int k = 99; k >= 0; --k) {
        const int t = k * 10, tn = (k - 1) * 10 < 0 ? -1 : (k - 1) * 10;
        const float at = s.ab[t + 1], an = s.ab[tn + 1];
        DdnmCoef c;
        c.sqrt_1m_at = sqrtf(1.0f - at); c.sqrt_at = sqrtf(at); c.sqrt_at_next = sqrtf(an);
        c.sigma_t = sqrtf(1.0f - an * an);
        c.c1 = sqrtf(1.0f - an) * (float)eta;
        c.c2 = sqrtf(1.0f - an) * (float)std::sqrt(1.0 - eta * eta);
        s.t.push_back(t); s.co.push_back(c);
    }
    return s;
}
__global__ void k_fill(float* p, float v, int n) { int i = blockIdx.x * blockDim.x + threadIdx.x; if (i < n) p[i] = v; }
}

extern "C" int pdhip_ddnm_schedule(float* at, float* at_next, int* t, int* t_next, float* coefs ) {
    Sched s = make_schedule();
    for (int k = 0; k < 100; ++k) {
        const int tt = s.t[k], tn = tt - 10 < 0 ? -1 : tt - 10;
        if (at) at[k] = s.ab[tt + 1];
        if (at_next) at_next[k] = s.ab[tn + 1];
        if (t) t[k] = tt;
        if (t_next) t_next[k] = tn;
        if (coefs) memcpy(coefs + 6 * k, &s.co[k], sizeof(DdnmCoef));
    }
    return PDHIP_OK;
}

extern "C" int pdhip_ddnm_step(float* x, const float* et, int et_channels, const float* y, const float* mask, const float* eps,
                               uint64_t seed, int step, int N, int HW, void* stream) {
    PD_REQUIRE(x && et && y && mask && step >= 0 && step < 100 && (et_channels == 3 || et_channels == 6), "pdhip_ddnm_step: bad arguments");
    static const Sched sched = make_schedule();
    return ddnm_update(x, et, et_channels, y, mask, eps, seed, (unsigned long long)step + 1, sched.co[step], N, HW, as_stream(stream));
}

extern "C" int pdhip_ddnm_prepare(const float* masked_imgs, const float* masks, float* y, int N, int HW, void* stream) {
    PD_REQUIRE(masked_imgs && masks && y, "pdhip_ddnm_prepare: null argument");
    return ddnm_prepare(masked_imgs, masks, y, N, HW, as_stream(stream));
}

extern "C" int pdhip_ddnm_sample_keyed(pdhip_unet* u, const float* masked_imgs, const float* masks, int N, const float* x_T,
                                       const float* eps_tape, uint64_t seed, uint64_t first_image_key, int n_steps, float* out,
                                       void* stream) {
    PD_REQUIRE(u && masked_imgs && masks && out, "pdhip_ddnm_sample: null argument");
    PD_REQUIRE(N >= 1 && N <= u->max_batch && n_steps >= 1 && n_steps <= 100, "pdhip_ddnm_sample: bad N / n_steps");
    static const Sched sched = make_schedule();
    hipStream_t s = as_stream(stream);
    const int HW = u->image_size * u->image_size;
    const long long n3 = (long long)N * 3 * HW;
    PD_TRY(ddnm_prepare(masked_imgs, masks, u->sy, N, HW, s));
    const unsigned long long quad0 = (unsigned long long)first_image_key * (unsigned long long)(3LL * HW / 4);
    if (x_T) PD_HIP(hipMemcpyAsync(u->sx, x_T, n3 * sizeof(float), hipMemcpyDeviceToDevice, s));
    else PD_TRY(philox_normal(u->sx, n3, seed, 0, s, quad0));
    if (u->steps_cached != n_steps) {
        PD_REQUIRE(u->have_te[0] && u->have_te[1] && u->have_te[2] && u->have_te[3], "unet: time_embed not loaded");
        float th[100];
        for (int k = 0; k < n_steps; ++k) th[k] = (float)sched.t[k];
        PD_HIP(hipMemcpyAsync(u->steps_t, th, n_steps * sizeof(float), hipMemcpyHostToDevice, s));
        PD_HIP(hipStreamSynchronize(s));
        PD_TRY(timestep_mlp(u->steps_t, n_steps, u->mc, u->te_w0, u->te_b0, u->te_w2, u->te_b2, u->steps_silu, u->steps_tmp, s));
        PD_TRY(gemv_rows(u->emb_w, u->emb_b, u->steps_silu, u->steps_emb, (int)u->emb_rows, u->ted, n_steps, s));
        u->steps_cached = n_steps;
    }
    const Tuning tun = tuning();
    for (int k = 0; k < n_steps; ++k) {
        PD_TRY(forward_impl(tun, u, u->sx, nullptr, N, u->set_, s, false, u->steps_emb + (size_t)k * u->emb_rows, 3));
        PD_TRY(ddnm_update(u->sx, u->set_, 3, u->sy, masks, eps_tape ? eps_tape + (size_t)k * n3 : nullptr, seed,
                           (unsigned long long)k + 1, sched.co[k], N, HW, s, quad0));
    }
    return ddnm_finish(u->sx, out, n3, s);
}
extern "C" int pdhip_ddnm_sample(pdhip_unet* u, const float* masked_imgs, const float* masks, int N, const float* x_T,
                                 const float* eps_tape, uint64_t seed, int n_steps, float* out, void* stream) {
    return pdhip_ddnm_sample_keyed(u, masked_imgs, masks, N, x_T, eps_tape, seed, 0, n_steps, out, stream);
}

static int swap_hook(int& field, int v) { const int old = field; field = v; return old; }
extern "C" int pdhip_debug_set_conv_tile(int wmw) { return swap_hook(tuning().force_wmw, wmw); }
extern "C" int pdhip_debug_set_conv_stages(int st) { return swap_hook(tuning().force_stages, st); }
extern "C" int pdhip_debug_set_conv_bk(int bk) { return swap_hook(tuning().force_bk, bk); }
extern "C" int pdhip_debug_set_conv_halo_strips(int mode) { return swap_hook(tuning().halo_strips, mode); }
extern "C" int pdhip_debug_set_conv_splitk(void* ws, long long ws_floats, int splits) {
    g_dbg_splitk_ws = (float*)ws; g_dbg_splitk_floats = ws ? (size_t)ws_floats : 0;
    if (ws != nullptr && ws_floats >= PD_SK_TICKET_FLOATS) (void)hipMemset(ws, 0, PD_SK_TICKET_FLOATS * sizeof(float));
    return swap_hook(tuning().force_splits, splits);
}
extern "C" int pdhip_debug_set_conv_sk(int mode, int tile, int splits) { tuning().sk_tile = tile; tuning().sk_splits = splits; return swap_hook(tuning().sk_mode, mode); }
extern "C" int pdhip_debug_set_conv_sk_stages(int stages) { return swap_hook(tuning().sk_stages, stages); }
extern "C" int pdhip_debug_set_conv_sk_kgroups(int kg) { return swap_hook(tuning().sk_kg, kg); }
extern "C" int pdhip_debug_set_conv_sk_order(int order) { return swap_hook(tuning().sk_order, order); }
extern "C" int pdhip_debug_set_conv_rr(int mode, int variant, int slabs) { tuning().rr_variant = variant; tuning().rr_slabs = slabs; return swap_hook(tuning().rr_mode, mode); }
extern "C" int pdhip_debug_set_conv_ht(int mode, int slabs) { tuning().ht_slabs = slabs; return swap_hook(tuning().ht_mode, mode); }
extern "C" int pdhip_debug_set_fuse_gn(int on) { return swap_hook(tuning().fuse_gn, on); }
extern "C" int pdhip_debug_set_fold_resample(int on) { return swap_hook(tuning().fold_resample, on); }
extern "C" int pdhip_debug_set_fold_skip(int on) { return swap_hook(tuning().fold_skip, on); }
extern "C" int pdhip_debug_set_rr_gn(int max_width) { return swap_hook(tuning().rr_gn, max_width); }
extern "C" int pdhip_debug_set_fold_finalize(int max_batch) { return swap_hook(tuning().fold_finalize, max_batch); }
extern "C" int pdhip_debug_set_fold_finalize_chunks(int chunks) { return swap_hook(tuning().fold_finalize_chunks, chunks); }
extern "C" int pdhip_debug_set_fuse_skip(int mode, int min_tiles) { if (min_tiles > 0) tuning().fuse_skip_min_tiles = min_tiles; return swap_hook(tuning().fuse_skip, mode); }
extern "C" int pdhip_debug_set_up_phase(int mode) { return swap_hook(tuning().up_phase, mode); }
extern "C" int pdhip_debug_set_attn(int nbuf, int vt_form, int qtiles) {
    Tuning& t = tuning();
    const int old = t.attn_nbuf | (t.attn_vt << 8) | (t.attn_qtn << 16);
    t.attn_nbuf = nbuf; t.attn_vt = vt_form; t.attn_qtn = qtiles;
    return old;
}
extern "C" int pdhip_debug_set_gn_iters(int iters) { return swap_hook(tuning().gn_iters, iters); }
extern "C" int pdhip_debug_set_gn_skip_variant(int v) { return swap_hook(tuning().gs_variant, v); }

extern "C" int pdhip_conv2d_nhwc_f16(const void* x, const void* w_packed, const float* bias, const void* residual, void* y,
                                     int N, int H, int W, int Cin, int Cout, int Cout_pad, int taps, const void* zero_page,
                                     void* stream) {
    PD_REQUIRE(x && w_packed && y && zero_page, "pdhip_conv2d_nhwc_f16: null argument");
    return conv_igemm(tuning(), (const half_t*)x, (const half_t*)w_packed, bias, (const half_t*)residual, (half_t*)y, N, H, W, Cin, Cout,
                      Cout_pad, taps, (const half_t*)zero_page, as_stream(stream), g_dbg_splitk_ws, g_dbg_splitk_floats);
}
extern "C" int pdhip_debug_conv_launch_nhwc_f16(const void* x, const void* x2, int Cin1, const void* w_packed, const float* bias, const void* residual,
                                                int res_up, const void* xs, const void* xs2, int Cs1, int Cs, void* y, int N, int H, int W, int Cin, int Cout,
                                                int Cout_pad, int taps, const void* zero_page, float* ws, long long ws_floats, float* gn_part,
                                                long long gn_part_floats, int* gn_chunks, int* kernel, void* stream) {
    const char* const fn = "pdhip_debug_conv_launch_nhwc_f16";
    PD_REQUIRE(x && w_packed && y && zero_page, "%s: null argument", fn);
    PD_REQUIRE(N > 0 && H > 0 && W > 0 && (taps == 1 || taps == 9), "%s: bad shape (N=%d H=%d W=%d taps=%d)", fn, N, H, W, taps);
    PD_REQUIRE(Cin % 32 == 0 && Cout % 8 == 0 && Cout_pad % 128 == 0 && Cout_pad >= Cout && Cin > 0 && Cout > 0,
               "%s: need Cin %% 32 == 0, Cout %% 8 == 0, padded Cout %% 128 == 0 (Cin=%d Cout=%d pad=%d)", fn, Cin, Cout, Cout_pad);
    PD_REQUIRE(x2 == nullptr || (taps == 1 && Cin1 > 0 && Cin1 < Cin && Cin1 % 64 == 0 && (Cin - Cin1) % 64 == 0),
               "%s: a two-source input needs a 1x1 conv and channel counts that are multiples of 64", fn);
    if (xs == nullptr) Cs = 0;
    PD_REQUIRE(xs == nullptr || (taps == 9 && Cs > 0 && Cs % 64 == 0 && (xs2 == nullptr || (Cs1 > 0 && Cs1 < Cs && Cs1 % 64 == 0))),
               "%s: a skip source needs a 3x3 conv and channel counts that are multiples of 64", fn);
    PD_REQUIRE(xs != nullptr || xs2 == nullptr, "%s: xs2 without xs", fn);
    PD_REQUIRE(xs == nullptr || residual == nullptr, "%s: the appended skip 1x1 takes the residual's place", fn);
    PD_REQUIRE(res_up == 0 || residual != nullptr, "%s: res_up without a residual", fn);
    const size_t wsf = ws != nullptr && ws_floats > 0 ? (size_t)ws_floats : 0;
    pdnn::ConvNeeds nd;
    nd.two_source = x2 != nullptr; nd.want_gn = gn_part != nullptr; nd.skip_cs = Cs;
    const pdnn::ConvPlan p = conv_plan(tuning(), N, H, W, Cin, Cout, Cout_pad, taps, nd, wsf);
    if (kernel) *kernel = (int)p.kernel;
    if (gn_chunks) *gn_chunks = p.gn_chunks;
    PD_REQUIRE(res_up == 0 || p.takes_res_up, "%s: the planned kernel (%s) does not read its residual at half resolution", fn, conv_kernel_name(p.kernel));
    PD_REQUIRE(Cs == 0 || p.takes_skip, "%s: the planned kernel (%s) does not append the skip 1x1", fn, conv_kernel_name(p.kernel));
    PD_REQUIRE(x2 == nullptr || p.kernel == pdnn::CONV_SK || p.kernel == pdnn::CONV_IGEMM, "%s: the planned kernel (%s) reads one source", fn,
               conv_kernel_name(p.kernel));
    PD_REQUIRE(gn_part == nullptr || gn_part_floats >= (long long)N * p.gn_chunks * (Cout / 8) * 2,
               "%s: gn_part holds %lld floats, the launch writes %lld", fn, gn_part_floats, (long long)N * p.gn_chunks * (Cout / 8) * 2);
    const pdnn::ConvArgs a{(const half_t*)x, (const half_t*)x2, x2 ? Cin1 : 0, (const half_t*)w_packed, bias, (const half_t*)residual, res_up, nullptr, nullptr,
                           (const half_t*)xs, (const half_t*)xs2, Cs1, (half_t*)y, (const half_t*)zero_page, wsf ? ws : nullptr, wsf, gn_part};
    return conv_launch(p, a, as_stream(stream));
}
extern "C" int pdhip_gn_finalize_oct_f32(const float* partA, int Ca, int chunksA, const float* partB, int Cb, int chunksB, int N, int HW, float* stats,
                                         void* stream) {
    PD_REQUIRE(partA && stats && N > 0 && HW > 0 && Ca > 0 && chunksA > 0, "pdhip_gn_finalize_oct_f32: bad arguments");
    PD_REQUIRE(partB ? (Cb > 0 && chunksB > 0) : Cb == 0, "pdhip_gn_finalize_oct_f32: partB and Cb / chunksB disagree");
    return gn_finalize_oct(partA, Ca, chunksA, partB, Cb, partB ? chunksB : 0, N, HW, 1e-5f, stats, as_stream(stream));
}
extern "C" int pdhip_pack_conv_up2_phase_f16(const void* w_packed, int Cin, int Cout_pad, void* w_phase, void* stream) {
    PD_REQUIRE(w_packed && w_phase && Cin > 0 && Cout_pad > 0, "pdhip_pack_conv_up2_phase_f16: bad arguments");
    return conv_up2_phase_pack((const half_t*)w_packed, Cin, Cout_pad, (half_t*)w_phase, as_stream(stream));
}
extern "C" int pdhip_conv3x3_up2_phase_nhwc_f16(const void* x, const void* w_phase, const float* bias, void* y, int N, int H, int W, int Cin, int Cout,
                                                int Cout_pad, const void* zero_page, float* gn_part, void* stream) {
    PD_REQUIRE(x && w_phase && y && zero_page, "pdhip_conv3x3_up2_phase_nhwc_f16: null argument");
    const pdnn::ConvPlan p = conv_up2_phase_plan(tuning(), N, 2 * H, 2 * W, Cin, Cout, Cout_pad, gn_part != nullptr);
    return conv_up2_phase((const half_t*)x, (const half_t*)w_phase, bias, (half_t*)y, N, H, W, Cin, Cout, Cout_pad, (const half_t*)zero_page,
                          as_stream(stream), p.gn_chunks > 0 ? gn_part : nullptr, p.geo);
}
extern "C" int pdhip_conv3x3_up2_halo_nhwc_f16(const void* x, const void* w_packed, const float* bias, void* y, int N, int H, int W, int Cin, int Cout,
                                               int Cout_pad, const void* zero_page, void* stream) {
    PD_REQUIRE(x && w_packed && y && zero_page, "pdhip_conv3x3_up2_halo_nhwc_f16: null argument");
    pdnn::ConvNeeds nd;
    nd.in_up = true;
    PD_REQUIRE(conv_plan(tuning(), N, 2 * H, 2 * W, Cin, Cout, Cout_pad, 9, nd, 0).takes_in_up,
               "pdhip_conv3x3_up2_halo_nhwc_f16: not a layer the halo-resident kernel takes unsplit");
    return conv_igemm(tuning(), (const half_t*)x, (const half_t*)w_packed, bias, nullptr, (half_t*)y, N, 2 * H, 2 * W, Cin, Cout, Cout_pad, 9,
                      (const half_t*)zero_page, as_stream(stream), nullptr, 0, nullptr, nullptr, 0, nullptr, 0, 1);
}
extern "C" int pdhip_gn_silu_skip1x1_nhwc_f16(const void* xa, const void* xb, int Ca, int C, const float* stats, const float* gamma,
                                              const float* beta, const void* w_packed, const float* bias, void* h0, void* sk, int N, int H,
                                              int W, void* stream) {
    PD_REQUIRE(xa && stats && gamma && beta && w_packed && h0 && sk, "pdhip_gn_silu_skip1x1_nhwc_f16: null argument");
    return gn_skip((const half_t*)xa, (const half_t*)xb, Ca, C, stats, gamma, beta, (const half_t*)w_packed, bias, (half_t*)h0, (half_t*)sk,
                   N, H * W, as_stream(stream), tuning().gs_variant);
}
extern "C" int pdhip_gn_silu_conv3x3_nhwc_f16(const void* x, const float* gamma, const float* beta, const float* film,
                                              long long film_stride, const void* w_packed, const float* bias, const void* residual,
                                              void* y, int N, int H, int W, int Cin, int Cout, int Cout_pad, const void* zero_page,
                                              float* ws, long long ws_floats, void* stream) {
    PD_REQUIRE(x && gamma && beta && w_packed && y && zero_page && ws, "pdhip_gn_silu_conv3x3_nhwc_f16: null argument");
    const size_t gws = (size_t)N * 64 * ((H * W + 255) / 256);
    PD_REQUIRE((size_t)ws_floats >= (size_t)N * 64 + gws + (size_t)N * Cin * 2, "pdhip_gn_silu_conv3x3_nhwc_f16: workspace too small");
    hipStream_t s = as_stream(stream);
    float* stats = ws;
    float* table = ws + (size_t)N * 64 + gws;
    PD_TRY(gn_stats((const half_t*)x, N, H * W, Cin, 1e-5f, stats, ws + (size_t)N * 64, gws, s));
    PD_TRY(gn_table(stats, gamma, beta, film, film_stride, N, Cin, table, s));
    float* hws = g_dbg_splitk_ws != nullptr && g_dbg_splitk_floats > PD_SK_TICKET_FLOATS ? g_dbg_splitk_ws + PD_SK_TICKET_FLOATS : nullptr;
    const size_t hws_floats = hws ? g_dbg_splitk_floats - PD_SK_TICKET_FLOATS : 0;
    PD_REQUIRE(conv3x3_halo_eligible(N, H, W, Cin, Cout_pad) && N > 0 && Cout > 0 && Cout_pad > 0, "conv3x3_halo: unsupported geometry (N=%d H=%d W=%d Cin=%d)", N, H, W, Cin);
    return conv3x3_halo((const half_t*)x, (const half_t*)w_packed, bias, (const half_t*)residual, (half_t*)y, N, H, W, Cin, Cout,
                        Cout_pad, (const half_t*)zero_page, s, nullptr, conv3x3_halo_launch_splits(tuning(), N, H, W, Cin, Cout, Cout_pad, hws_floats),
                        conv3x3_halo_rows(tuning(), H, W), hws, hws_floats, table);
}
extern "C" int pdhip_debug_conv3x3_apply(const void* x, const float* table, const void* w_packed, const float* bias, const void* residual,
                                         void* y, int N, int H, int W, int Cin, int Cout, int Cout_pad, const void* zero_page, void* stream) {
    PD_REQUIRE(x && table && w_packed && y && zero_page, "pdhip_debug_conv3x3_apply: null argument");
    return conv3x3_halo((const half_t*)x, (const half_t*)w_packed, bias, (const half_t*)residual, (half_t*)y, N, H, W, Cin, Cout,
                        Cout_pad, (const half_t*)zero_page, as_stream(stream), nullptr, 1, conv3x3_halo_rows(tuning(), H, W), nullptr, 0, table);
}
extern "C" int pdhip_pack_conv_weight_f16(const float* w_oihw, int Cout, int Cin, int taps, void* w_packed, void* stream) {
    PD_REQUIRE(w_oihw && w_packed, "pdhip_pack_conv_weight_f16: null argument");
    k_pack_conv<<<grid_for((long long)Cout * Cin * taps), 256, 0, as_stream(stream)>>>(w_oihw, 0, Cout, Cin, taps, (half_t*)w_packed);
    PD_LAUNCH_CHECK();
    return PDHIP_OK;
}
extern "C" int pdhip_groupnorm_nhwc_f16(const void* x, const float* gamma, const float* beta, const float* film, int N, int H,
                                        int W, int C, int silu, int resample, void* y, float* stats_ws ,
                                        float* ws, long long ws_floats, void* stream) {
    PD_REQUIRE(x && gamma && beta && y && stats_ws && ws, "pdhip_groupnorm_nhwc_f16: null argument");
    PD_TRY(gn_stats((const half_t*)x, N, H * W, C, 1e-5f, stats_ws, ws, (size_t)ws_floats, as_stream(stream)));
    return gn_apply((const half_t*)x, stats_ws, gamma, beta, film, 2LL * C, N, H, W, C, silu, resample, y, 0, as_stream(stream), nullptr, 0, nullptr, nullptr,
                    tuning().gn_iters);
}
extern "C" size_t pdhip_unet_head_ws_floats(int N, int H, int W, int C, int Cout) {
    return (size_t)N * 64 + (size_t)N * 64 * ((H * W + 255) / 256) + (size_t)Cout * 9 * C + (size_t)64 * C;
}
extern "C" int pdhip_unet_head_f32(const void* x, const float* gamma, const float* beta, const float* w_oihw, const float* bias,
                                   int N, int H, int W, int C, int Cout, float* y_nchw, float* ws, long long ws_floats, void* stream) {
    PD_REQUIRE(x && gamma && beta && w_oihw && bias && y_nchw && ws, "pdhip_unet_head_f32: null argument");
    PD_REQUIRE((size_t)ws_floats >= pdhip_unet_head_ws_floats(N, H, W, C, Cout), "pdhip_unet_head_f32: workspace too small");
    hipStream_t s = as_stream(stream);
    float* stats = ws;
    float* gws = stats + (size_t)N * 64;
    const size_t gws_floats = (size_t)N * 64 * ((H * W + 255) / 256);
    float* wp = gws + gws_floats;
    half_t* wz = reinterpret_cast<half_t*>(wp + (size_t)Cout * 9 * C);
    PD_TRY(gn_stats((const half_t*)x, N, H * W, C, 1e-5f, stats, gws, gws_floats, s));
    k_pack_conv_f32<<<grid_for((long long)Cout * 9 * C), 256, 0, s>>>(w_oihw, 0, Cout, C, 9, wp);
    PD_LAUNCH_CHECK();
    PD_TRY(head_pack(wp, Cout, C, wz, s));
    return head_gn_silu_conv3x3((const half_t*)x, stats, gamma, beta, wz, bias, y_nchw, N, H, W, C, Cout, s);
}
extern "C" int pdhip_attention_f16(const void* qkv, void* out, int N, int T, int C, int head_dim, void* vt_ws, void* stream) {
    PD_REQUIRE(qkv && out, "pdhip_attention_f16: null argument");
    const Tuning& t = tuning();
    return attention((const half_t*)qkv, (half_t*)out, N, T, C, head_dim, as_stream(stream), (half_t*)vt_ws, t.attn_nbuf, t.attn_qtn, t.attn_vt);
}
extern "C" int pdhip_philox_normal(float* out, long long n, uint64_t seed, uint64_t stream_id, void* stream) {
    PD_REQUIRE(out && n > 0, "pdhip_philox_normal: bad arguments");
    return philox_normal(out, n, seed, stream_id, as_stream(stream));
}
extern "C" int pdhip_bench_copy16(const void* src, void* dst, long long bytes, int blocks, int unroll, void* stream) {
    return copy16(src, dst, bytes, blocks, unroll, as_stream(stream));
}
extern "C" int pdhip_gn_apply_f16(const void* x, const void* x2, int Ca, int C, const float* stats, const float* partA, int chunksA,
                                  const float* partB, int chunksB, const float* gamma, const float* beta, const float* film,
                                  long long film_stride, int N, int H, int W, int silu, int resample, void* y, void* y_raw, void* stream) {
    PD_REQUIRE(x && gamma && beta && y, "pdhip_gn_apply_f16: null argument");
    PD_REQUIRE(N > 0 && H > 0 && W > 0 && C > 0, "pdhip_gn_apply_f16: empty tensor");
    PD_REQUIRE((stats != nullptr) != (partA != nullptr), "pdhip_gn_apply_f16: the statistics come finished (stats) or as octet partials (partA), not both");
    PD_REQUIRE(stats == nullptr || (partB == nullptr && chunksA == 0 && chunksB == 0), "pdhip_gn_apply_f16: partials next to finished statistics");
    PD_REQUIRE(partA == nullptr || (chunksA >= 1 && (x2 == nullptr ? (partB == nullptr && chunksB == 0) : (partB != nullptr && chunksB >= 1))),
               "pdhip_gn_apply_f16: one set of octet partials (and a chunk count >= 1) per source tensor");
    PD_REQUIRE(film == nullptr || film_stride >= 2LL * C, "pdhip_gn_apply_f16: film rows hold scale[C] | shift[C]");
    if (partA != nullptr) {
        const GnPartsArg pa{partA, x2 ? Ca : C, chunksA, partB, x2 ? C - Ca : 0, chunksB, 1e-5f};
        return gn_apply((const half_t*)x, nullptr, gamma, beta, film, film_stride, N, H, W, C, silu, resample, y, 0, as_stream(stream),
                        (const half_t*)x2, x2 ? Ca : 0, (half_t*)y_raw, &pa, tuning().gn_iters);
    }
    return gn_apply((const half_t*)x, stats, gamma, beta, film, film_stride, N, H, W, C, silu, resample, y, 0, as_stream(stream),
                    (const half_t*)x2, x2 ? Ca : 0, (half_t*)y_raw, nullptr, tuning().gn_iters);
}
extern "C" int pdhip_gn_table_f32(const float* stats, const float* gamma, const float* beta, const float* film, long long film_stride, int N, int C,
                                  float* table, void* stream) {
    PD_REQUIRE(stats && gamma && beta && table && N > 0 && C > 0, "pdhip_gn_table_f32: bad arguments");
    PD_REQUIRE(film == nullptr || film_stride >= 2LL * C, "pdhip_gn_table_f32: film rows hold scale[C] | shift[C]");
    return gn_table(stats, gamma, beta, film, film_stride, N, C, table, as_stream(stream));
}
extern "C" int pdhip_resample2x_nhwc_f16(const void* x, int N, int H, int W, int C, int mode, void* y, void* stream) {
    PD_REQUIRE(x && y && N > 0 && H > 0 && W > 0 && C > 0, "pdhip_resample2x_nhwc_f16: bad arguments");
    PD_REQUIRE(mode != 1 || (H % 2 == 0 && W % 2 == 0), "pdhip_resample2x_nhwc_f16: avgpool needs even H, W");
    return resample2x((const half_t*)x, N, H, W, C, mode, (half_t*)y, as_stream(stream));
}
extern "C" int pdhip_concat_channels_f16(const void* a, int Ca, const void* b, int Cb, long long pixels, void* y, void* stream) {
    PD_REQUIRE(a && b && y && Ca > 0 && Cb > 0 && pixels > 0, "pdhip_concat_channels_f16: bad arguments");
    return concat_channels((const half_t*)a, Ca, (const half_t*)b, Cb, pixels, (half_t*)y, as_stream(stream));
}
```

pointdreamer_amd/ddnm_inpainting.py:

```python
import ctypes as C
import math
import os

import torch

from . import _lib
from ._lib import ptr, stream, check

_reg = _lib.register
vp, i32, i64, f32, f64, u64 = C.c_void_p, C.c_int, C.c_int64, C.c_float, C.c_double, C.c_uint64
_reg('pdhip_unet_create', C.c_int, [i32, i32, i32, C.POINTER(C.c_int), i32, C.POINTER(C.c_int), i32, i32, i32, i32,
                                    C.POINTER(vp)])
_reg('pdhip_unet_destroy', None, [vp])
_reg('pdhip_unet_arena_bytes', C.c_longlong, [vp])
_reg('pdhip_unet_num_tensors', C.c_int, [vp])
_reg('pdhip_unet_load_tensor', C.c_int, [vp, C.c_char_p, vp, i32, C.POINTER(C.c_int64), i32, vp])
_reg('pdhip_unet_missing_tensors', C.c_int, [vp, C.c_char_p, i32])
_reg('pdhip_unet_forward', C.c_int, [vp, vp, vp, i32, vp, vp])
_reg('pdhip_unet_profile', C.c_int, [vp, i32])
_reg('pdhip_unet_profile_read', C.c_int, [vp, C.POINTER(C.c_double), C.POINTER(C.c_double), C.POINTER(C.c_longlong)])
_reg('pdhip_unet_profile_read_attention', C.c_int, [vp, C.POINTER(C.c_double), C.POINTER(C.c_double), C.POINTER(C.c_longlong)])
_reg('pdhip_ddnm_schedule', C.c_int, [vp, vp, vp, vp, vp])
_reg('pdhip_ddnm_prepare', C.c_int, [vp, vp, vp, i32, i32, vp])
_reg('pdhip_ddnm_step', C.c_int, [vp, vp, i32, vp, vp, vp, u64, i32, i32, i32, vp])
_reg('pdhip_ddnm_sample', C.c_int, [vp, vp, vp, i32, vp, vp, u64, i32, vp, vp])
_reg('pdhip_ddnm_sample_keyed', C.c_int, [vp, vp, vp, i32, vp, vp, u64, u64, i32, vp, vp])
_reg('pdhip_debug_set_conv_bk', C.c_int, [i32])
_reg('pdhip_debug_set_conv_stages', C.c_int, [i32])
_reg('pdhip_debug_set_conv_tile', C.c_int, [i32])
_reg('pdhip_debug_set_conv_halo_strips', C.c_int, [i32])
_reg('pdhip_debug_set_conv_splitk', C.c_int, [vp, C.c_longlong, i32])
_reg('pdhip_pack_conv_weight_f16', C.c_int, [vp, i32, i32, i32, vp, vp])
_reg('pdhip_unet_head_ws_floats', C.c_size_t, [i32, i32, i32, i32, i32])
_reg('pdhip_unet_head_f32', C.c_int, [vp, vp, vp, vp, vp, i32, i32, i32, i32, i32, vp, vp, C.c_longlong, vp])
_reg('pdhip_conv2d_nhwc_f16', C.c_int, [vp, vp, vp, vp, vp, i32, i32, i32, i32, i32, i32, i32, vp, vp])
_reg('pdhip_groupnorm_nhwc_f16', C.c_int, [vp, vp, vp, vp, i32, i32, i32, i32, i32, i32, vp, vp, vp, C.c_longlong, vp])
_reg('pdhip_gn_silu_conv3x3_nhwc_f16', C.c_int, [vp, vp, vp, vp, C.c_longlong, vp, vp, vp, vp, i32, i32, i32, i32, i32, i32, vp, vp, C.c_longlong, vp])
_reg('pdhip_debug_set_fuse_gn', C.c_int, [i32])
_reg('pdhip_gn_silu_skip1x1_nhwc_f16', C.c_int, [vp, vp, i32, i32, vp, vp, vp, vp, vp, vp, vp, i32, i32, i32, vp])
_reg('pdhip_debug_set_fuse_skip', C.c_int, [i32, i32])
_reg('pdhip_debug_set_gn_skip_variant', C.c_int, [i32])
_reg('pdhip_debug_set_fold_resample', C.c_int, [i32])
_reg('pdhip_debug_set_fold_finalize', C.c_int, [i32])
_reg('pdhip_debug_set_fold_finalize_chunks', C.c_int, [i32])
_reg('pdhip_debug_set_fold_skip', C.c_int, [i32])
_reg('pdhip_debug_set_up_phase', C.c_int, [i32])
_reg('pdhip_pack_conv_up2_phase_f16', C.c_int, [vp, i32, i32, vp, vp])
_reg('pdhip_conv3x3_up2_phase_nhwc_f16', C.c_int, [vp, vp, vp, vp, i32, i32, i32, i32, i32, i32, vp, vp, vp])
_reg('pdhip_conv3x3_up2_halo_nhwc_f16', C.c_int, [vp, vp, vp, vp, i32, i32, i32, i32, i32, i32, vp, vp])
_reg('pdhip_debug_set_conv_sk', C.c_int, [i32, i32, i32])
_reg('pdhip_debug_set_conv_sk_stages', C.c_int, [i32])
_reg('pdhip_debug_set_conv_sk_kgroups', C.c_int, [i32])
_reg('pdhip_debug_set_conv_sk_order', C.c_int, [i32])
_reg('pdhip_debug_set_attn', C.c_int, [i32, i32, i32])
_reg('pdhip_debug_set_conv_rr', C.c_int, [i32, i32, i32])
_reg('pdhip_debug_set_rr_gn', C.c_int, [i32])
_reg('pdhip_debug_set_conv_ht', C.c_int, [i32, i32])
_reg('pdhip_conv_ht_plan', C.c_int, [i32, i32, i32, i32, i32, i32, C.c_longlong, C.POINTER(C.c_int), C.POINTER(C.c_int)])
_reg('pdhip_unet_route_table', C.c_int, [i32, i32, i32, C.POINTER(C.c_int), i32, C.POINTER(C.c_int), i32, i32, i32, i32, i32, C.c_char_p, i32])
_reg('pdhip_conv_ht_f16', C.c_int, [vp, vp, vp, vp, i32, vp, i32, i32, i32, i32, i32, i32, vp, vp, C.c_longlong, vp, C.POINTER(C.c_int), vp])
_reg('pdhip_conv_rr_weight_halfs', C.c_longlong, [i32, i32, i32, i32])
_reg('pdhip_conv_rr_pack_f16', C.c_int, [vp, i32, i32, i32, i32, vp, vp])
_reg('pdhip_gn_octet_partials_f16', C.c_int, [vp, i32, i32, i32, i32, vp, vp])
_reg('pdhip_gn_apply_parts_f16', C.c_int, [vp, vp, i32, i32, vp, i32, vp, i32, vp, vp, vp, C.c_longlong, i32, i32, i32, i32, vp, vp])
_reg('pdhip_conv_rr_f16', C.c_int, [vp, vp, i32, i32, i32, vp, vp, vp, C.c_longlong, vp, i32, vp, i32, vp, vp, i32, i32, i32, vp, vp, vp, i32, vp,
                                   i32, i32, i32, i32, vp, C.c_longlong, vp, C.POINTER(C.c_int), vp])
_reg('pdhip_debug_conv_launch_nhwc_f16', C.c_int, [vp, vp, i32, vp, vp, vp, i32, vp, vp, i32, i32, vp, i32, i32, i32, i32, i32, i32, i32, vp, vp, C.c_longlong,
                                                  vp, C.c_longlong, C.POINTER(C.c_int), C.POINTER(C.c_int), vp])
_reg('pdhip_gn_finalize_oct_f32', C.c_int, [vp, i32, i32, vp, i32, i32, i32, i32, vp, vp])
_reg('pdhip_debug_conv3x3_apply', C.c_int, [vp, vp, vp, vp, vp, vp, i32, i32, i32, i32, i32, i32, vp, vp])
_reg('pdhip_attention_f16', C.c_int, [vp, vp, i32, i32, i32, i32, vp, vp])
_reg('pdhip_philox_normal', C.c_int, [vp, C.c_longlong, u64, u64, vp])
_reg('pdhip_gemv_rows_f32', C.c_int, [vp, vp, vp, vp, i32, i32, i32, i32, vp])
_reg('pdhip_timestep_mlp_f32', C.c_int, [vp, i32, i32, vp, vp, vp, vp, vp, vp, vp])
_reg('pdhip_conv_in_f16', C.c_int, [vp, vp, vp, vp, i32, i32, i32, i32, i32, vp, vp, vp])
_reg('pdhip_debug_set_gn_iters', C.c_int, [i32])
_reg('pdhip_gn_apply_f16', C.c_int, [vp, vp, i32, i32, vp, vp, i32, vp, i32, vp, vp, vp, C.c_longlong, i32, i32, i32, i32, i32, vp, vp, vp])
_reg('pdhip_gn_table_f32', C.c_int, [vp, vp, vp, vp, C.c_longlong, i32, i32, vp, vp])
_reg('pdhip_resample2x_nhwc_f16', C.c_int, [vp, i32, i32, i32, i32, i32, vp, vp])
_reg('pdhip_concat_channels_f16', C.c_int, [vp, i32, vp, i32, C.c_longlong, vp, vp])
_reg('pdhip_bench_copy16', C.c_int, [vp, vp, C.c_longlong, i32, i32, vp])

IMAGENET_256 = dict(image_size=256, num_channels=256, num_res_blocks=2, attention_resolutions="32,16,8",
                    num_head_channels=64, learn_sigma=True, use_scale_shift_norm=True, resblock_updown=True,
                    use_fp16=True, channel_mult="")
DEFAULT_CKPT = 'models/DDNM/256x256_diffusion_uncond.pt'


def default_channel_mult(image_size):
    return {512: (0.5, 1, 1, 2, 2, 4, 4), 256: (1, 1, 2, 2, 4, 4), 128: (1, 1, 2, 3, 4), 64: (1, 2, 3, 4)}[image_size]


def unet_route_table(N, image_size=256, num_channels=256, num_res_blocks=2, attention_resolutions="32,16,8", num_head_channels=64,
                     learn_sigma=True, channel_mult="", max_batch=64, **unused):
    L = _lib.lib()
    cm = tuple(int(c) for c in channel_mult.split(",")) if channel_mult else default_channel_mult(image_size)
    ads = tuple(image_size // int(r) for r in attention_resolutions.split(","))
    args = (image_size, num_channels, num_res_blocks, (C.c_int * len(cm))(*cm), len(cm), (C.c_int * len(ads))(*ads), len(ads), num_head_channels,
            6 if learn_sigma else 3, max_batch, N)
    n = L.pdhip_unet_route_table(*args, None, 0)
    check(min(n, 0), 'pdhip_unet_route_table')
    buf = C.create_string_buffer(n + 1)
    check(min(L.pdhip_unet_route_table(*args, buf, n + 1), 0), 'pdhip_unet_route_table')
    return buf.value.decode().splitlines()


class UNetModel:

    def __init__(self, image_size=256, num_channels=256, num_res_blocks=2, attention_resolutions="32,16,8",
                 num_head_channels=64, learn_sigma=True, channel_mult="", max_batch=8, device='cuda', **unused):
        if not unused.get('use_scale_shift_norm', True) or not unused.get('resblock_updown', True):
            raise NotImplementedError("only the scale-shift-norm / resblock-updown variant (imagenet_256.yml) is built")
        L = _lib.lib()
        cm = tuple(int(c) for c in channel_mult.split(",")) if channel_mult else default_channel_mult(image_size)
        if any(int(c) != c for c in cm):
            raise NotImplementedError("fractional channel multipliers (image_size 512) are not built")
        ads = tuple(image_size // int(r) for r in attention_resolutions.split(","))
        self.image_size, self.out_channels, self.max_batch = image_size, 6 if learn_sigma else 3, max_batch
        self.device = _lib.resolve_device(device)
        cm_arr = (C.c_int * len(cm))(*[int(c) for c in cm])
        ad_arr = (C.c_int * len(ads))(*ads)
        h = vp()
        with torch.cuda.device(self.device):
            check(L.pdhip_unet_create(image_size, num_channels, num_res_blocks, cm_arr, len(cm), ad_arr, len(ads),
                                      num_head_channels, self.out_channels, max_batch, C.byref(h)), 'pdhip_unet_create')
        self._h = h
        self._L = L

    def __del__(self):
        h, self._h = getattr(self, '_h', None), None
        if h:
            self._L.pdhip_unet_destroy(h)

    @property
    def arena_bytes(self):
        return int(self._L.pdhip_unet_arena_bytes(self._h))

    def load_state_dict(self, state_dict, strict=True):
        L = self._L
        n = 0
        with torch.cuda.device(self.device):
            for name, t in state_dict.items():
                if t.dtype not in (torch.float32, torch.float16):
                    t = t.float()
                t = t.to(self.device).contiguous()
                shape = (C.c_int64 * t.dim())(*t.shape)
                rc = L.pdhip_unet_load_tensor(self._h, name.encode(), ptr(t), 1 if t.dtype == torch.float16 else 0, shape,
                                              t.dim(), stream())
                if rc == -5 and not strict:
                    continue
                check(rc, f'pdhip_unet_load_tensor({name})')
                n += 1
            torch.cuda.synchronize(self.device)
        buf = C.create_string_buffer(4096)
        missing = L.pdhip_unet_missing_tensors(self._h, buf, 4096)
        if strict and missing:
            raise _lib.PdhipError(f"load_state_dict: {missing} tensors missing, e.g. {buf.value.decode().split()[:4]}")
        return n

    def forward(self, x, timesteps):
        x = x.float().contiguous()
        t = timesteps.float().to(x.device).contiguous()
        N = x.shape[0]
        if x.device != self.device:
            raise _lib.PdhipError(f"UNetModel lives on {self.device}, input is on {x.device}")
        out = torch.empty((N, self.out_channels, self.image_size, self.image_size), device=x.device)
        with torch.cuda.device(self.device):
            check(self._L.pdhip_unet_forward(self._h, ptr(x), ptr(t), N, ptr(out), stream()), 'pdhip_unet_forward')
        return out

    __call__ = forward

    def profile(self, enable):
        check(self._L.pdhip_unet_profile(self._h, int(enable)), 'pdhip_unet_profile')

    def profile_read(self, attention=False):
        ms, fl, n = C.c_double(), C.c_double(), C.c_longlong()
        fn = self._L.pdhip_unet_profile_read_attention if attention else self._L.pdhip_unet_profile_read
        check(fn(self._h, C.byref(ms), C.byref(fl), C.byref(n)), 'pdhip_unet_profile_read')
        return ms.value, fl.value, n.value


def ddnm_schedule():
    import numpy as np
    L = _lib.lib()
    at = np.zeros(100, np.float32)
    an = np.zeros(100, np.float32)
    t = np.zeros(100, np.int32)
    tn = np.zeros(100, np.int32)
    co = np.zeros((100, 6), np.float32)
    check(L.pdhip_ddnm_schedule(at.ctypes.data, an.ctypes.data, t.ctypes.data, tn.ctypes.data, co.ctypes.data),
          'pdhip_ddnm_schedule')
    return at, an, t, tn, co


def random_state_dict(model_kwargs, seed=0, device='cpu'):
    image_size = model_kwargs.get('image_size', 256)
    mc = model_kwargs.get('num_channels', 256)
    nres = model_kwargs.get('num_res_blocks', 2)
    cm = model_kwargs.get('channel_mult') or ""
    cm = tuple(int(c) for c in cm.split(",")) if cm else default_channel_mult(image_size)
    ads = tuple(image_size // int(r) for r in model_kwargs.get('attention_resolutions', "32,16,8").split(","))
    out_ch = 6 if model_kwargs.get('learn_sigma', True) else 3
    ted = mc * 4
    g = torch.Generator(device='cpu').manual_seed(seed)
    sd = {}

    def lin(name, o, i):
        sd[name + '.weight'] = torch.randn((o, i), generator=g) / math.sqrt(i)
        sd[name + '.bias'] = torch.randn((o,), generator=g) * 0.05

    def conv(name, o, i, k, one_d=False):
        shape = (o, i, k) if one_d else (o, i, k, k)
        sd[name + '.weight'] = torch.randn(shape, generator=g) / math.sqrt(i * k * (1 if one_d else k))
        sd[name + '.bias'] = torch.randn((o,), generator=g) * 0.05

    def norm(name, c):
        sd[name + '.weight'] = 1.0 + torch.randn((c,), generator=g) * 0.05
        sd[name + '.bias'] = torch.randn((c,), generator=g) * 0.05

    def res(name, cin, cout):
        norm(name + '.in_layers.0', cin); conv(name + '.in_layers.2', cout, cin, 3)
        lin(name + '.emb_layers.1', 2 * cout, ted)
        norm(name + '.out_layers.0', cout); conv(name + '.out_layers.3', cout, cout, 3)
        if cin != cout:
            conv(name + '.skip_connection', cout, cin, 1)

    def att(name, c):
        norm(name + '.norm', c); conv(name + '.qkv', 3 * c, c, 1, True); conv(name + '.proj_out', c, c, 1, True)
    lin('time_embed.0', ted, mc); lin('time_embed.2', ted, ted)
    ch = int(cm[0] * mc)
    conv('input_blocks.0.0', ch, 3, 3)
    chans = [ch]
    ds, n = 1, 1
    for level, mult in enumerate(cm):
        for _ in range(nres):
            res(f'input_blocks.{n}.0', ch, int(mult * mc)); ch = int(mult * mc)
            if ds in ads:
                att(f'input_blocks.{n}.1', ch)
            chans.append(ch); n += 1
        if level != len(cm) - 1:
            res(f'input_blocks.{n}.0', ch, ch); chans.append(ch); ds *= 2; n += 1
    res('middle_block.0', ch, ch); att('middle_block.1', ch); res('middle_block.2', ch, ch)
    n = 0
    for level, mult in list(enumerate(cm))[::-1]:
        for i in range(nres + 1):
            ich = chans.pop()
            res(f'output_blocks.{n}.0', ch + ich, int(mc * mult)); ch = int(mc * mult)
            k = 1
            if ds in ads:
                att(f'output_blocks.{n}.{k}', ch); k += 1
            if level and i == nres:
                res(f'output_blocks.{n}.{k}', ch, ch); ds //= 2
            n += 1
    norm('out.0', ch); conv('out.2', out_ch, ch, 3)
    return {k: v.to(device) for k, v in sd.items()}


class Inpainter:

    def __init__(self, device, ckpt_path=DEFAULT_CKPT, model_kwargs=None, max_batch=8, allow_random_weights=False,
                 seed=1234, state_dict=None):
        self.device = _lib.resolve_device(device)
        kw = dict(IMAGENET_256)
        kw.update(model_kwargs or {})
        self.model = UNetModel(max_batch=max_batch, device=self.device, **kw)
        if state_dict is None:
            if ckpt_path and os.path.exists(ckpt_path):
                state_dict = torch.load(ckpt_path, map_location='cpu')
            elif allow_random_weights:
                state_dict = random_state_dict(kw, seed=0)
            else:
                raise FileNotFoundError(f"{ckpt_path} not found (the reference downloads it; there is no network here). "
                                        "Pass allow_random_weights=True for a random-weight run.")
        self.model.load_state_dict(state_dict, strict=True)
        self.seed = seed
        self.n_steps = 100
        self._images = 0
        self.max_batch = max_batch

    def inpaint_views(self, masked_imgs, masks, x_T=None, eps_tape=None, n_steps=None, first_key=None, advance=None):
        L = _lib.lib()
        masked_imgs = masked_imgs.float().contiguous()
        masks = masks.float().contiguous()
        V = masked_imgs.shape[0]
        out = torch.empty_like(masked_imgs)
        steps = int(n_steps or self.n_steps)
        key0 = self._images if first_key is None else int(first_key)
        with torch.cuda.device(self.device):
            for s in range(0, V, self.max_batch):
                e = min(V, s + self.max_batch)
                xt = None if x_T is None else x_T[s:e].float().contiguous()
                tape = None if eps_tape is None else eps_tape[:, s:e].float().contiguous()
                check(L.pdhip_ddnm_sample_keyed(self.model._h, ptr(masked_imgs[s:e]), ptr(masks[s:e]), e - s, ptr(xt, allow_none=True),
                                                ptr(tape, allow_none=True), self.seed, key0 + s, steps, ptr(out[s:e]),
                                                stream()), 'pdhip_ddnm_sample')
        self._images = (key0 + V) if advance is None else (self._images + int(advance))
        return out

    def inpaint(self, masked_imgs, masks):
        imgs = masked_imgs.permute(0, 3, 1, 2).contiguous()
        return self.inpaint_views(imgs, masks[:, :, :, 0].contiguous())
```

Before: 2215 shapes/hour.

## Run up-sampling phase convolution through the halo-tiled conv kernel with four taps

Adds a four-tap variant of the LDS halo conv3x3 kernel that computes one of the four sub-pixel phases of an upsample-by-2 conv per tile, then scatters outputs to interleaved positions and emits per-phase GroupNorm partials for both 256-pixel halves. The plan routes upsample convs to it when the source width is 128 and batch is at least 8, or when forced. The aim is to reuse the halo kernel's staged input tile and pipelining for the decoder's largest upsample convs instead of the older phase kernel. The cost is more kernel complexity, extra template instantiations, and a second GroupNorm reduction pass in the epilogue.

```diff
diff --git a/include/pdhip.h b/include/pdhip.h
--- a/include/pdhip.h
+++ b/include/pdhip.h
@@ -232,6 +232,8 @@
                               void* y, int N, int H, int W, int Cin, int Cout, int Cout_pad, const void* zero_page, void* stream);
 int pdhip_debug_set_fold_skip(int on);
 int pdhip_debug_set_up_phase(int mode);
+int pdhip_debug_set_up_phase_halo(int mode);
+int pdhip_debug_up2_phase_geo(int N, int H, int W, int Cin, int Cout, int Cout_pad);
 int pdhip_pack_conv_up2_phase_f16(const void* w_packed, int Cin, int Cout_pad, void* w_phase, void* stream);
 int pdhip_conv3x3_up2_phase_nhwc_f16(const void* x, const void* w_phase, const float* bias, void* y, int N, int H, int W, int Cin, int Cout,
                                      int Cout_pad, const void* zero_page, float* gn_part, void* stream);
diff --git a/pointdreamer_amd/csrc/nn_common.h b/pointdreamer_amd/csrc/nn_common.h
--- a/pointdreamer_amd/csrc/nn_common.h
+++ b/pointdreamer_amd/csrc/nn_common.h
@@ -33,6 +33,7 @@
     int fold_finalize = 8, fold_finalize_chunks = 16;
     int fuse_skip = 1, fuse_skip_min_tiles = 1;
     int up_phase = 1;
+    int up_phase_halo = 1;
     int attn_nbuf = 0;
     int attn_qtn = 0;
     int attn_vt = 0;
@@ -59,6 +60,9 @@
                int res_up = 0,
                int in_up = 0);
 bool conv_up2_phase_eligible(int N, int H, int W, int Cin, int Cout, int Cout_pad);
+bool conv_up2_phase_halo_eligible(int N, int H, int W, int Cin, int Cout, int Cout_pad);
+int conv_up2_phase_halo(const half_t* X, const half_t* Wph, const float* bias, half_t* Y, int N, int H, int W, int Cin, int Cout, int Cout_pad,
+                        const half_t* zero_page, hipStream_t s, float* gn_part);
 int conv_up2_phase_pack(const half_t* w9, int Cin, int Cout_pad, half_t* dst, hipStream_t s);
 int conv_up2_phase(const half_t* X, const half_t* Wph, const float* bias, half_t* Y, int N, int H, int W, int Cin, int Cout, int Cout_pad,
                    const half_t* zero_page, hipStream_t s, float* gn_part, int geo);
diff --git a/pointdreamer_amd/csrc/nn_conv_halo.hip b/pointdreamer_amd/csrc/nn_conv_halo.hip
--- a/pointdreamer_amd/csrc/nn_conv_halo.hip
+++ b/pointdreamer_amd/csrc/nn_conv_halo.hip
@@ -14,7 +14,7 @@
 __device__ __forceinline__ int swz_b(int row) { return (0x78 >> (2 * ((row >> 2) & 3))) & 3; }
 __device__ __forceinline__ int swz_a(int hp) { return ((hp >> 2) & 1) << 1; }
 
-template <int WLOG, int ILOG, bool APPLY>
+template <int WLOG, int ILOG, bool APPLY, int TAPS = 9>
 __global__ __launch_bounds__(512) void k_conv3x3_halo(const half_t* __restrict__ X, const half_t* __restrict__ Wt,
                                                       const float* __restrict__ bias, const half_t* __restrict__ residual,
                                                       half_t* __restrict__ Y, int N, int H, int Cin, int Cout, int n_tiles,
@@ -28,8 +28,12 @@
     constexpr int RPW = W >= 128 ? 1 : 128 / W;
     constexpr int FPR = TM / RPW;
     constexpr int CS_LD = BNT + 8;
-    static_assert(PA <= 9 && RPW <= 4, "halo schedule: at most one halo piece per wave per tap, W >= 32");
+    constexpr int NT = TAPS;
+    static_assert(TAPS == 9 || TAPS == 4, "nine taps, or the four of one up-sampling phase");
+    static_assert(PA <= 9 && RPW <= 4, "halo schedule: at most one halo piece per wave per tap (4 taps: three in steps 0-2), W >= 32");
     static_assert(!APPLY || PA <= 7, "APPLY: piece T-1 is finished under step T+1 <= 8");
+    static_assert(TAPS == 9 || PA <= 8, "phase form: step 3 issues no halo piece (and the PA == 9 prologue order is the 9-tap one)");
+    static_assert(TAPS == 9 || (!APPLY && ILOG == WLOG), "phase form: plain input, full-row tiles (its halves are the 256-pixel GroupNorm chunks)");
     constexpr int SCR_OFF = 2 * AH_BYTES + 3 * B_BYTES;
     constexpr int TAB_OFF = SCR_OFF + NWAVES * 1024;
     extern __shared__ __attribute__((aligned(16))) char smem[];
@@ -41,14 +45,20 @@
         const int b = blockIdx.x, q = total_tiles >> 3, r = total_tiles & 7, xcd = b & 7, i = b >> 3;
         tile = (xcd < r ? xcd * (q + 1) : r * (q + 1) + (xcd - r) * q) + i;
     }
-    const int pt = tile / n_tiles, n0 = (tile % n_tiles) * BNT;
+    int pt = tile / n_tiles;
+    const int n0 = (tile % n_tiles) * BNT;
+    int phase = 0;
+    if constexpr (TAPS == 4) {
+        phase = pt & 3; pt >>= 2;
+        Wt += (size_t)phase * ((size_t)n_tiles * BNT) * (4 * Cin);
+    }
     const int HWp = H << ILOG;
     const int tpi = HWp / BMT;
     const int img = pt / tpi, tin = pt - img * tpi;
     constexpr int STRIPS = 1 << (ILOG - WLOG);
     const int ty0 = (tin / STRIPS) * RT, x0 = (tin % STRIPS) << WLOG;
     auto pix = [&](int p) -> long long { return (((long long)img * H + ty0 + (p >> WLOG)) << ILOG) + x0 + (p & (W - 1)); };
-    const int K = 9 * Cin;
+    const int K = NT * Cin;
     const int NCT = Cin >> 5;
     const int cb = (int)((long long)NCT * blockIdx.y / splits), NC = (int)((long long)NCT * (blockIdx.y + 1) / splits) - cb;
 
@@ -87,7 +97,7 @@
     const int r16 = lane & 15, q4 = lane >> 4;
     const uint32_t lds0 = (uint32_t)(uintptr_t)(__attribute__((address_space(3))) char*)smem;
     const int p0 = wm * 128;
-    const int hp0 = ((p0 >> WLOG) + 1) * HW2 + (p0 & (W - 1)) + 1 + r16;
+    const int hp0 = ((p0 >> WLOG) + 1) * HW2 + (p0 & (W - 1)) + 1 + r16 + (TAPS == 4 ? (phase >> 1) * HW2 + (phase & 1) : 0);
     const uint32_t b_frag = lds0 + 2 * AH_BYTES + (wn * 64 + r16) * ROWB + ((q4 ^ swz_b(r16)) << 4);
     float4_t acc[TM][4];
 #pragma unroll
@@ -200,18 +210,21 @@
     int bs = 0;
     uint32_t a_carry;
     { const int hpv = hp0; a_carry = HL_AADDR(0, -HW2 - 1, 0); }
-    const int S = 9 * NC;
+    const int S = NT * NC;
     for (int c0 = 0; c0 < NC; c0 += 2) {
+#define HL_NP4(T) ((T) == 3 ? 0 : (PA - 3 * (T) < 0 ? 0 : PA - 3 * (T) > 3 ? 3 : PA - 3 * (T)))
 #ifdef PD_LAB_AP_LOOSEVM
-#define HL_VMN(T) (1 + ((T) < PA ? 1 : 0) + (((((T) + 8) % 9) < PA) ? 1 : 0))
+#define HL_VMN9(T) (1 + ((T) < PA ? 1 : 0) + (((((T) + 8) % 9) < PA) ? 1 : 0))
 #else
-#define HL_VMN(T) (1 + ((T) < PA ? 1 : 0) + ((!APPLY && (((T) + 8) % 9) < PA) ? 1 : 0))
-#endif
+#define HL_VMN9(T) (1 + ((T) < PA ? 1 : 0) + ((!APPLY && (((T) + 8) % 9) < PA) ? 1 : 0))
+#endif
+#define HL_VMN(T) (TAPS == 9 ? HL_VMN9(T) : (T) == 3 ? 1 : 1 + HL_NP4(T) + HL_NP4(((T) + 3) & 3))
+#define HL_TOFF(T) (TAPS == 9 ? ((T) / 3 - 1) * HW2 + ((T) % 3 - 1) : (((T) >> 1) - 1) * HW2 + (((T) & 1) - 1))
 #define HL_GROUP(P, T, g)                                                                                              \
     {                                                                                                                 \
         if constexpr ((g) + 3 < TM) {                                  \
             if constexpr (RPW > 1 && ((g) == 0 || ((g) + 3) % FPR == 0 || RPW == 2))                                  \
-                a_cur = HL_AADDR(ab, (T / 3 - 1) * HW2 + (T % 3 - 1), ((g) + 3) / FPR);                               \
+                a_cur = HL_AADDR(ab, HL_TOFF(T), ((g) + 3) / FPR);                                                    \
             HL_DSR(ar[((g) + 3) & 3], a_cur, (((g) + 3) % FPR) * 1024);                                               \
         }                                                                                                             \
         if constexpr ((g) == 5) {                                                                                     \
@@ -220,7 +233,7 @@
                 __builtin_amdgcn_s_barrier();                                                                         \
                 asm volatile("" ::: "memory");                                                                        \
                 const uint32_t b_nx = b_frag + (bs == 2 ? 0 : bs + 1) * B_BYTES;                                      \
-                a_nx0 = HL_AADDR(abn, dyn_ * HW2 + dxn_, 0);                                                          \
+                a_nx0 = HL_AADDR(abn, HL_TOFF(tn_), 0);                                                               \
                 a_carry = a_nx0;                                                                                      \
                 HL_DSR(bf[bn][0], b_nx, 0); HL_DSR(bf[bn][1], b_nx, 16 * ROWB);                                       \
                 HL_DSR(bf[bn][2], b_nx, 32 * ROWB); HL_DSR(bf[bn][3], b_nx, 48 * ROWB);                               \
@@ -236,7 +249,7 @@
             if (more) HL_DSR(ar[1], a_nx0, 1024);                                                                     \
         } else if constexpr ((g) == 7) {                                                                              \
             if (more) {                                                                                               \
-                if constexpr (FPR == 2) a_nx0 = HL_AADDR(abn, dyn_ * HW2 + dxn_, 1);                                  \
+                if constexpr (FPR == 2) a_nx0 = HL_AADDR(abn, HL_TOFF(tn_), 1);                                       \
                 HL_DSR(ar[2], a_nx0, (2 % FPR) * 1024);                                                               \
             }                                                                                                         \
         } else {                                                                                                      \
@@ -255,44 +268,51 @@
             const int st2 = bs == 0 ? 2 : bs - 1;                                                                     \
             if (s + 2 < S) {                                                                                          \
                 glds16h(bp, b_dst + st2 * B_BYTES);                                                                   \
-                if constexpr (((T) + 2) % 9 < 8) bp += Cin; else bp += 32 - 8 * Cin;                                  \
+                if constexpr (((T) + 2) % NT < NT - 1) bp += Cin; else bp += 32 - (NT - 1) * Cin;                            \
             } else glds16h(zero_page, b_dst + st2 * B_BYTES);            \
         }                                                                                                             \
-        if constexpr ((g) == 1 && (T) < PA) {                                          \
+        if constexpr (TAPS == 9 && (g) == 1 && (T) < PA) {                             \
             glds16h(halo_src(T, cb + min(c + 1, NC - 1)), ah_dst + piece_off(T, ab ^ 1));                            \
         }                                                                                                             \
+        if constexpr (TAPS == 4 && (g) >= 1 && (g) <= 3 && (T) < 3 && 3 * (T) + (g) - 1 < PA) {    \
+            glds16h(halo_src(3 * (T) + (g) - 1, cb + min(c + 1, NC - 1)), ah_dst + piece_off(3 * (T) + (g) - 1, ab ^ 1)); \
+        }                                                                                                             \
         __builtin_amdgcn_sched_barrier(0);                                                                            \
     }
 #define HL_STEP(P, T)                                                                                                 \
     {                                                                                                                 \
-        constexpr int tn_ = ((T) + 1) % 9;                                                                            \
-        constexpr int dyn_ = tn_ / 3 - 1, dxn_ = tn_ % 3 - 1;                                                         \
-        constexpr int ab = (P), bc = ((P) + (T)) & 1, bn = bc ^ 1;     \
-        const int s = c * 9 + (T);                                                                                    \
+        constexpr int tn_ = ((T) + 1) % NT;                                                                           \
+        constexpr int ab = (P), bc = ((P) * NT + (T)) & 1, bn = bc ^ 1;     \
+        const int s = c * NT + (T);                                                                                   \
         const bool more = s + 1 < S;                                                                                  \
         int hpv = hp0;                                                                                                \
         asm volatile("" : "+v"(hpv));                                  \
         uint32_t a_cur = a_carry;                                      \
-        const int abn = (T) == 8 ? (ab ^ 1) : ab;                                                                     \
+        const int abn = (T) == NT - 1 ? (ab ^ 1) : ab;                                                                 \
         uint32_t a_nx0 = 0;                                            \
         HL_GROUP(P, T, 0) HL_GROUP(P, T, 1) HL_GROUP(P, T, 2) HL_GROUP(P, T, 3)                                        \
         HL_GROUP(P, T, 4) HL_GROUP(P, T, 5) HL_GROUP(P, T, 6) HL_GROUP(P, T, 7)                                        \
         bs = bs == 2 ? 0 : bs + 1;                                                                                    \
     }
-#define HL_CHUNK(P) HL_STEP(P, 0) HL_STEP(P, 1) HL_STEP(P, 2) HL_STEP(P, 3) HL_STEP(P, 4) HL_STEP(P, 5) HL_STEP(P, 6) HL_STEP(P, 7) HL_STEP(P, 8)
+#define HL_CHUNK(P)                                                                                                   \
+    HL_STEP(P, 0) HL_STEP(P, 1) HL_STEP(P, 2) HL_STEP(P, 3)                                                           \
+    if constexpr (TAPS == 9) { HL_STEP(P, 4) HL_STEP(P, 5) HL_STEP(P, 6) HL_STEP(P, 7) HL_STEP(P, 8) }
         { const int c = c0; HL_CHUNK(0) }
         if (c0 + 1 < NC) { const int c = c0 + 1; HL_CHUNK(1) }
 #undef HL_CHUNK
 #undef HL_STEP
 #undef HL_GROUP
+#undef HL_TOFF
 #undef HL_VMN
+#undef HL_VMN9
+#undef HL_NP4
     }
 #undef HL_AADDR
 #undef HL_DSR
     asm volatile("s_waitcnt vmcnt(0)" ::: "memory");
     __syncthreads();
 
-    if (partial != nullptr) {
+    if (TAPS == 9 && partial != nullptr) {
         const long long M = (long long)N * HWp;
         float* P = partial + (size_t)blockIdx.y * (size_t)M * Cout;
 #pragma unroll
@@ -314,6 +334,7 @@
     constexpr int RPP = NWAVES * 64 / CT;
     const int col8 = (tid % CT) * 8;
     float gs = 0.f, gq = 0.f;
+    float gs2 = 0.f, gq2 = 0.f;
     auto epilogue = [&](auto has_res) {
         constexpr bool RES = decltype(has_res)::value;
         float4_t bvs[4];
@@ -359,7 +380,9 @@
 #pragma unroll
         for (int p = 0; p < BMT / RPP; ++p) {
             const int row = p * RPP + tid / CT;
-            const long long m = pix(row);
+            long long m = pix(row);
+            if constexpr (TAPS == 4)
+                m = (((long long)img * 2 * H + 2 * (ty0 + (row >> WLOG)) + (phase >> 1)) << (ILOG + 1)) + 2 * (x0 + (row & (W - 1))) + (phase & 1);
             half8 v = *reinterpret_cast<const half8*>(&Cs[row * CS_LD + col8]);
             const size_t o = (size_t)m * Cout + n0 + col8;
             if (RES) {
@@ -372,7 +395,10 @@
                 *reinterpret_cast<half8*>(Y + o) = v;
 #endif
 #pragma unroll
-                for (int e = 0; e < 8; ++e) { const float f = (float)v[e]; gs += f; gq += f * f; }
+                for (int e = 0; e < 8; ++e) {
+                    const float f = (float)v[e];
+                    if (TAPS == 4 && p >= BMT / RPP / 2) { gs2 += f; gq2 += f * f; } else { gs += f; gq += f * f; }
+                }
             }
         }
     };
@@ -381,34 +407,40 @@
     if (gs == 123.456f && gq == 7.f) Y[0] = (half_t)1.f;
 #endif
     if (gn_part != nullptr) {
-        __syncthreads();
-        float* red = reinterpret_cast<float*>(smem);
-        red[tid * 2] = gs; red[tid * 2 + 1] = gq;
-        __syncthreads();
-        constexpr int SUB = 8;
-        static_assert(RPP % SUB == 0, "GroupNorm partial reduce");
-        float* red2 = red + NWAVES * 64 * 2;
-        if (tid < CT * SUB) {
-            const int j = tid % SUB, c = tid / SUB;
-            float s1 = 0.f, q1 = 0.f;
-#pragma unroll
-            for (int r = 0; r < RPP / SUB; ++r) { s1 += red[((r * SUB + j) * CT + c) * 2]; q1 += red[((r * SUB + j) * CT + c) * 2 + 1]; }
-            red2[tid * 2] = s1; red2[tid * 2 + 1] = q1;
-        }
-        __syncthreads();
-        if (tid < CT && n0 + tid * 8 < Cout) {
-            float s1 = 0.f, q1 = 0.f;
-#pragma unroll
-            for (int j = 0; j < SUB; ++j) { s1 += red2[(tid * SUB + j) * 2]; q1 += red2[(tid * SUB + j) * 2 + 1]; }
-            const int chunks = tpi;
-            const int chunk = tin;
-            float* dst = gn_part + (((size_t)img * chunks + chunk) * (Cout >> 3) + (n0 >> 3) + tid) * 2;
-            dst[0] = s1; dst[1] = q1;
-        }
-    }
-}
-
-template <int WLOG, int ILOG, bool APPLY>
+        auto gn_reduce = [&](float ps, float pq, int chunks, int chunk) {
+            __syncthreads();
+            float* red = reinterpret_cast<float*>(smem);
+            red[tid * 2] = ps; red[tid * 2 + 1] = pq;
+            __syncthreads();
+            constexpr int SUB = 8;
+            static_assert(RPP % SUB == 0, "GroupNorm partial reduce");
+            float* red2 = red + NWAVES * 64 * 2;
+            if (tid < CT * SUB) {
+                const int j = tid % SUB, c = tid / SUB;
+                float s1 = 0.f, q1 = 0.f;
+#pragma unroll
+                for (int r = 0; r < RPP / SUB; ++r) { s1 += red[((r * SUB + j) * CT + c) * 2]; q1 += red[((r * SUB + j) * CT + c) * 2 + 1]; }
+                red2[tid * 2] = s1; red2[tid * 2 + 1] = q1;
+            }
+            __syncthreads();
+            if (tid < CT && n0 + tid * 8 < Cout) {
+                float s1 = 0.f, q1 = 0.f;
+#pragma unroll
+                for (int j = 0; j < SUB; ++j) { s1 += red2[(tid * SUB + j) * 2]; q1 += red2[(tid * SUB + j) * 2 + 1]; }
+                float* dst = gn_part + (((size_t)img * chunks + chunk) * (Cout >> 3) + (n0 >> 3) + tid) * 2;
+                dst[0] = s1; dst[1] = q1;
+            }
+        };
+        if constexpr (TAPS == 4) {
+            gn_reduce(gs, gq, tpi * 8, (tin * 2) * 4 + phase);
+            gn_reduce(gs2, gq2, tpi * 8, (tin * 2 + 1) * 4 + phase);
+        } else {
+            gn_reduce(gs, gq, tpi, tin);
+        }
+    }
+}
+
+template <int WLOG, int ILOG, bool APPLY, int TAPS = 9>
 int launch_halo_v(const half_t* X, const half_t* Wt, const float* bias, const half_t* residual, half_t* Y, int N, int H, int Cin,
                   int Cout, int Cout_pad, const half_t* zero_page, hipStream_t s, float* gn_part, int splits, float* partial,
                   const float* ap_table, int res_up, int in_up) {
@@ -416,10 +448,10 @@
     const size_t loop_bytes = (size_t)2 * NPA * 1024 + 3 * 8192 + (APPLY ? (size_t)8 * 1024 + (size_t)Cin * 8 + (size_t)NPA * 16 + 16 : 0);
     const size_t smem = std::max<size_t>(loop_bytes, (size_t)512 * (128 + 8) * 2);
     PD_REQUIRE(smem <= 160 * 1024, "conv3x3_halo: %zu bytes of LDS (Cin = %d)", smem, Cin);
-    auto kern = k_conv3x3_halo<WLOG, ILOG, APPLY>;
+    auto kern = k_conv3x3_halo<WLOG, ILOG, APPLY, TAPS>;
     PD_HIP(hipFuncSetAttribute((const void*)kern, hipFuncAttributeMaxDynamicSharedMemorySize, (int)smem));
     const int n_tiles = Cout_pad / 128;
-    const int total = (int)(((long long)N * H * (1 << ILOG)) / 512) * n_tiles;
+    const int total = (int)(((long long)N * H * (1 << ILOG)) / 512) * (TAPS == 4 ? 4 : 1) * n_tiles;
     kern<<<dim3(total, splits), 512, smem, s>>>(X, Wt, bias, residual, Y, N, H, Cin, Cout, n_tiles, total, zero_page, gn_part, splits,
                                                 partial, ap_table, res_up, in_up);
     return PDHIP_OK;
@@ -492,4 +524,20 @@
     return PDHIP_OK;
 }
 
-}
+bool conv_up2_phase_halo_eligible(int N, int H, int W, int Cin, int Cout, int Cout_pad) {
+    return (W == 32 || W == 64 || W == 128) && conv3x3_halo_eligible(N, H, W, Cin, Cout_pad) && Cout % 8 == 0 && Cout_pad >= Cout &&
+           ((long long)N * H * W / 512) * 4 * (Cout_pad / 128) < (1LL << 30);
+}
+int conv_up2_phase_halo(const half_t* X, const half_t* Wph, const float* bias, half_t* Y, int N, int H, int W, int Cin, int Cout,
+                        int Cout_pad, const half_t* zero_page, hipStream_t s, float* gn_part) {
+    PD_REQUIRE(conv_up2_phase_halo_eligible(N, H, W, Cin, Cout, Cout_pad),
+               "conv_up2_phase_halo: unsupported geometry (N=%d H=%d W=%d Cin=%d Cout=%d pad=%d)", N, H, W, Cin, Cout, Cout_pad);
+#define HL_PHASE(WL) launch_halo_v<WL, WL, false, 4>(X, Wph, bias, nullptr, Y, N, H, Cin, Cout, Cout_pad, zero_page, s, gn_part, 1, nullptr, nullptr, 0, 0)
+    const int rc = W == 128 ? HL_PHASE(7) : W == 64 ? HL_PHASE(6) : HL_PHASE(5);
+#undef HL_PHASE
+    if (rc) return rc;
+    PD_LAUNCH_CHECK();
+    return PDHIP_OK;
+}
+
+}
diff --git a/pointdreamer_amd/csrc/nn_gemm.hip b/pointdreamer_amd/csrc/nn_gemm.hip
--- a/pointdreamer_amd/csrc/nn_gemm.hip
+++ b/pointdreamer_amd/csrc/nn_gemm.hip
@@ -598,11 +598,18 @@
     return done(CONV_IGEMM);
 }
 
+static bool up_phase_halo_wins(int N, int Ws) {
+    return N >= 8 && Ws == 128;
+}
+
 ConvPlan conv_up2_phase_plan(const Tuning& t, int N, int H, int W, int Cin, int Cout, int Cout_pad, bool want_gn) {
     ConvPlan p;
     p.N = N; p.H = H; p.W = W; p.Cin = Cin; p.Cout = Cout; p.Cout_pad = Cout_pad; p.taps = 9;
     p.kernel = CONV_UP_PHASE; p.want_gn = want_gn;
     p.geo = Cout_pad % 256 != 0 || t.force_wmw == 16 ? 16 : 8;
+    if (t.up_phase_halo != 0 && t.force_wmw == 0 && conv_up2_phase_halo_eligible(N, H / 2, W / 2, Cin, Cout, Cout_pad) &&
+        (t.up_phase_halo == 2 || up_phase_halo_wins(N, W / 2)))
+        p.geo = 512;
     p.gn_chunks = want_gn && ((long long)H * W / 4) % 256 == 0 ? (int)((long long)H * W / 256) : 0;
     return p;
 }
@@ -723,6 +730,8 @@
 }
 int conv_up2_phase(const half_t* X, const half_t* Wph, const float* bias, half_t* Y, int N, int H, int W, int Cin, int Cout, int Cout_pad,
                    const half_t* zero_page, hipStream_t s, float* gn_part, int geo) {
+    if (geo == 512)
+        return conv_up2_phase_halo(X, Wph, bias, Y, N, H, W, Cin, Cout, Cout_pad, zero_page, s, gn_part);
     PD_REQUIRE(conv_up2_phase_eligible(N, H, W, Cin, Cout, Cout_pad),
                "conv_up2_phase: need Cin %% 64 == 0, Cout %% 8 == 0, padded Cout %% 128 == 0 (Cin=%d Cout=%d pad=%d)", Cin, Cout, Cout_pad);
     PD_REQUIRE(geo == 16 || (geo == 8 && Cout_pad % 256 == 0), "conv_up2_phase: no plan (geo=%d)", geo);
diff --git a/pointdreamer_amd/csrc/nn_unet.hip b/pointdreamer_amd/csrc/nn_unet.hip
--- a/pointdreamer_amd/csrc/nn_unet.hip
+++ b/pointdreamer_amd/csrc/nn_unet.hip
@@ -932,6 +932,7 @@
 extern "C" int pdhip_debug_set_fold_finalize_chunks(int chunks) { return swap_hook(tuning().fold_finalize_chunks, chunks); }
 extern "C" int pdhip_debug_set_fuse_skip(int mode, int min_tiles) { if (min_tiles > 0) tuning().fuse_skip_min_tiles = min_tiles; return swap_hook(tuning().fuse_skip, mode); }
 extern "C" int pdhip_debug_set_up_phase(int mode) { return swap_hook(tuning().up_phase, mode); }
+extern "C" int pdhip_debug_set_up_phase_halo(int mode) { return swap_hook(tuning().up_phase_halo, mode); }
 extern "C" int pdhip_debug_set_attn(int nbuf, int vt_form, int qtiles) {
     Tuning& t = tuning();
     const int old = t.attn_nbuf | (t.attn_vt << 8) | (t.attn_qtn << 16);
@@ -998,6 +999,9 @@
     return conv_up2_phase((const half_t*)x, (const half_t*)w_phase, bias, (half_t*)y, N, H, W, Cin, Cout, Cout_pad, (const half_t*)zero_page,
                           as_stream(stream), p.gn_chunks > 0 ? gn_part : nullptr, p.geo);
 }
+extern "C" int pdhip_debug_up2_phase_geo(int N, int H, int W, int Cin, int Cout, int Cout_pad) {
+    return conv_up2_phase_plan(tuning(), N, 2 * H, 2 * W, Cin, Cout, Cout_pad, false).geo;
+}
 extern "C" int pdhip_conv3x3_up2_halo_nhwc_f16(const void* x, const void* w_packed, const float* bias, void* y, int N, int H, int W, int Cin, int Cout,
                                                int Cout_pad, const void* zero_page, void* stream) {
     PD_REQUIRE(x && w_packed && y && zero_page, "pdhip_conv3x3_up2_halo_nhwc_f16: null argument");
diff --git a/pointdreamer_amd/ddnm_inpainting.py b/pointdreamer_amd/ddnm_inpainting.py
--- a/pointdreamer_amd/ddnm_inpainting.py
+++ b/pointdreamer_amd/ddnm_inpainting.py
@@ -45,6 +45,8 @@
 _reg('pdhip_debug_set_fold_finalize_chunks', C.c_int, [i32])
 _reg('pdhip_debug_set_fold_skip', C.c_int, [i32])
 _reg('pdhip_debug_set_up_phase', C.c_int, [i32])
+_reg('pdhip_debug_set_up_phase_halo', C.c_int, [i32])
+_reg('pdhip_debug_up2_phase_geo', C.c_int, [i32, i32, i32, i32, i32, i32])
 _reg('pdhip_pack_conv_up2_phase_f16', C.c_int, [vp, i32, i32, vp, vp])
 _reg('pdhip_conv3x3_up2_phase_nhwc_f16', C.c_int, [vp, vp, vp, vp, i32, i32, i32, i32, i32, i32, vp, vp, vp])
 _reg('pdhip_conv3x3_up2_halo_nhwc_f16', C.c_int, [vp, vp, vp, vp, i32, i32, i32, i32, i32, i32, vp, vp])
```

After: 2217 shapes/hour (median of 6 runs). No clear change (+0.1%).
